# rslmtoasa/rslmtoasa

Hardware: AMD Instinct MI355X
Metric: block-recursion throughput (H|psi> + A_n + B_n recursion levels, recursion.f90 recur_b) (higher is better)
Workload: dtype f64

## Files before the change

### rslmtoasa_amd/csrc/kernels_spmm5.hpp

```cpp
#pragma once
#include <hip/hip_runtime.h>
#include <algorithm>
#include <type_traits>
#include <utility>
#include <vector>
#include "kernels_valu.hpp"
#include "kernels_mfma.hpp"
#include "kernels_spmm4.hpp"

namespace rsrec {

#ifndef RSREC_S5_KSPLIT_PROBE
#define RSREC_S5_KSPLIT_PROBE 0
#endif
#ifndef RSREC_S5_PRIO
#define RSREC_S5_PRIO 0
#endif
#ifndef RSREC_S5_GRAM_STRIP_LOADS
#define RSREC_S5_GRAM_STRIP_LOADS 0
#endif
#ifndef S5_WG_GROUPS
#define S5_WG_GROUPS 4
#endif
constexpr int S5_TRIPLE = 640;
// ... 182 lines not shown
                if ((int)E.size() > nextra) {
                    Head& H = head_main[(size_t)set * ntau + tau];
                    H.blk.assign(E[nextra].blk, E[nextra].blk + 2 * BLK); H.flip = 0; H.valid = true;
                }
                for (int sig = 0; sig < 2; ++sig)
                    emit_stream(E, sig, 0, (9 * (int)E.size() + 9) / 10, host.data() + set * per_set + ((size_t)tau * 2 + sig) * per_sig);
            }
        if (hipMemcpy(d_frag, host.data(), host.size() * sizeof(double), hipMemcpyHostToDevice) != hipSuccess) return "upload of spmm5 fragments failed";
        return nullptr;
    }
    void emit_head(int set, int tau, const double* extra, double* out) const {
        const Head& H = head_main[(size_t)set * ntau + tau];
        std::vector<Entry> E = {{extra, nslots, 0}, {extra, nslots, 1}};
        if (H.valid) E.push_back({H.blk.data(), 0, H.flip});
        for (int sig = 0; sig < 2; ++sig) emit_stream(E, sig, 0, S5_HEAD_TRIPLES, out + (size_t)sig * S5_HEAD_TRIPLES * S5_TRIPLE);
    }
    const char* build(int nslots_lat, int hstride, int ntype, int nmax, int hoh, const double* st, const double* loc, const double* eeo, const double* hallo,
                      const double* enim, const double* lsham, const int* iz0, const double* const* dev = nullptr, hipStream_t stream = nullptr) {
        const int nt = nmax + ntype, nset = hoh ? 2 : 1, nfs = nslots_lat + 1;
        const size_t B = 2 * (size_t)BLK;
        std::vector<const double*> blk((size_t)nset * nt * nfs, nullptr);
        const size_t tmp_per = dev ? 1 : (size_t)nfs;
        std::vector<double> tmp((size_t)(hoh ? nt : 0) * tmp_per * B, 0.0);
        std::vector<S5Desc> desc(dev ? (size_t)nset * nt * nfs : 0, S5Desc{nullptr, nullptr, 1.0, 0.0});
        for (int tau = 0; tau < nt; ++tau)
            for (int s = 0; s < nslots_lat; ++s) {
                const size_t off = tau < nmax ? B * (s + (size_t)hstride * tau) : B * (s + (size_t)hstride * (tau - nmax));
                const double* h0 = (tau < nmax ? loc : st) + off;
                blk[(size_t)tau * nfs + s] = h0;
                if (dev) desc[(size_t)tau * nfs + s] = S5Desc{(tau < nmax ? dev[1] : dev[0]) + off, nullptr, 1.0, 0.0};
                if (hoh) {
                    const double* ho = (tau < nmax ? hallo : eeo) + off;
                    if (dev) { blk[((size_t)nt + tau) * nfs + s] = ho; desc[((size_t)nt + tau) * nfs + s] = S5Desc{(tau < nmax ? dev[3] : dev[2]) + off, nullptr, -1.0, s == 0 ? 1.0 : 0.0}; }
                    else {
                        double* d = tmp.data() + B * ((size_t)tau * tmp_per + s);
                        for (size_t e = 0; e < B; ++e) d[e] = -ho[e];
                        if (s == 0) for (int q = 0; q < NB; ++q) d[2 * (q + NB * q)] += 1.0;
                        blk[((size_t)nt + tau) * nfs + s] = d;
                    }
                }
            }
        if (hoh)
            for (int tau = 0; tau < nt; ++tau) {
                const int ty = tau < nmax ? iz0[tau] : tau - nmax;
                double* d = tmp.data() + B * ((size_t)tau * tmp_per + (dev ? 0 : nslots_lat));
                for (size_t e = 0; e < B; ++e) d[e] = enim[B * ty + e] + lsham[B * ty + e];
                blk[((size_t)nt + tau) * nfs + nslots_lat] = d;
                if (dev) desc[((size_t)nt + tau) * nfs + nslots_lat] = S5Desc{dev[4] + B * ty, dev[5] + B * ty, 1.0, 0.0};
            }
        if (!dev) return build_custom(nslots_lat, nt, nset, blk);
        if (const char* msg = make_schedule(nslots_lat, nt, nset, kinds_of(blk), nullptr)) return msg;
        head_main.assign((size_t)nset * nt, Head());
        const size_t dneed = desc.size() * sizeof(S5Desc);
        if (dneed > desc_bytes) {
            if (d_desc) (void)hipFree(d_desc);
            d_desc = nullptr; desc_bytes = 0;
            if (hipMalloc(reinterpret_cast<void**>(&d_desc), dneed) != hipSuccess) return "hipMalloc of spmm5 block descriptors failed";
            desc_bytes = dneed;
        }
        if (hipMemcpyAsync(d_desc, desc.data(), dneed, hipMemcpyHostToDevice, stream) != hipSuccess) return "upload of spmm5 block descriptors failed";
        if (hipStreamSynchronize(stream) != hipSuccess) return "upload of spmm5 block descriptors failed";
        k_s5_emit<<<dim3(ntr, 2, nset * nt), S5_TRIPLE, 0, stream>>>(d_desc, d_meta, META, nfs, nslots_lat + 1, ntr, d_frag);
        if (hipGetLastError() != hipSuccess) return "launch of the operator-stream assembly failed";
        return nullptr;
    }
    int single_class(int set) const {
        int one = -1;
        for (int tau = 0; tau < ntau; ++tau)
            if (ksteps[(size_t)set * ntau + tau] > 0) { if (one >= 0) return -1; one = tau; }
        return one;
    }
    double required_flops(int set, int tau, int slot) const {
        const size_t q = ((size_t)set * ntau + tau) * (nslots + 1) + slot;
        if (q >= mixing.size() || mixing[q] < 0) return 0.0;
        return mixing[q] ? 46656.0 : 23328.0;
    }
    double flops_per_group(int set, int tau) const { return ksteps.empty() ? 0.0 : 2.0 * ksteps[(size_t)set * ntau + tau] * 9.0 * (2.0 * 16 * 16 * 4 + 2.0 * 4 * 4 * 4 * 4); }
    const double* frag_set(int set) const { return d_frag + (size_t)set * ntau * 2 * ntr * S5_TRIPLE; }
    const int* meta_set(int set) const { return d_meta + (size_t)set * ntau * META; }
};

typedef double s5_d2 __attribute__((ext_vector_type(2)));
struct S5Pair { s5_d2 b[9]; s5_d2 a[2]; };
struct S5Single { double b[9]; double a[2]; };
struct S5Acc { double4_t m[9]; double r[9]; };

struct S5Ent { unsigned off[GROUP]; unsigned rem; };

template <int S> struct S5St {
    static constexpr int T = S / 3, K = S % 3;
    static constexpr int W = K == 2 ? 2 : 4;
    static constexpr int o0 = 10 * T + (K == 0 ? 0 : K == 1 ? 4 : 8);
    static constexpr int eA = o0 / 9, mA0 = o0 % 9, sp = 9 - mA0;
    static constexpr bool straddle = sp < W;
    static constexpr bool opens = straddle || mA0 == 0;
    static constexpr int eOpen = mA0 == 0 ? eA : eA + 1;
};

template <int NL, int NM>
__device__ __forceinline__ void s5_interleave() {
    constexpr int PER = NM / NL;
#pragma unroll
    for (int i = 0; i < NL; ++i) {
        __builtin_amdgcn_sched_group_barrier(0x20, 1, 0);
        __builtin_amdgcn_sched_group_barrier(0x8, PER, 0);
    }
    __builtin_amdgcn_sched_group_barrier(0x8, NM - PER * NL, 0);
}

template <int NL = 11>
__device__ __forceinline__ void s5_mfma(S5Acc& acc, const S5Pair& o) {
#pragma unroll
    for (int e = 0; e < 2; ++e)
#pragma unroll
        for (int t = 0; t < 9; ++t) {
            acc.m[t] = __builtin_amdgcn_mfma_f64_16x16x4f64(o.a[0][e], o.b[t][e], acc.m[t], 0, 0, 0);
            acc.r[t] = __builtin_amdgcn_mfma_f64_4x4x4f64(o.a[1][e], o.b[t][e], acc.r[t], 0, 0, 0);
        }
    s5_interleave<NL, 36>();
}
template <int NL = 11>
__device__ __forceinline__ void s5_mfma(S5Acc& acc, const S5Single& o) {
#pragma unroll
    for (int t = 0; t < 9; ++t) {
        acc.m[t] = __builtin_amdgcn_mfma_f64_16x16x4f64(o.a[0], o.b[t], acc.m[t], 0, 0, 0);
        acc.r[t] = __builtin_amdgcn_mfma_f64_4x4x4f64(o.a[1], o.b[t], acc.r[t], 0, 0, 0);
    }
    s5_interleave<NL, 18>();
}

template <int N> using S5C = std::integral_constant<int, N>;
template <int T0, int... I, class F>
__device__ __forceinline__ void s5_each_tile(std::integer_sequence<int, I...>, F&& f) { (f(S5C<T0 + I>{}, S5C<I>{}), ...); }
template <int SRC>
__device__ __forceinline__ s5_d2 s5_row_bcast(s5_d2 v) {
    s5_d2 r;
#pragma unroll
    for (int c = 0; c < 2; ++c) {
        const int lo = __builtin_amdgcn_update_dpp(0, __double2loint(v[c]), 0x150 + SRC , 0xf, 0xf, true);
        const int hi = __builtin_amdgcn_update_dpp(0, __double2hiint(v[c]), 0x150 + SRC, 0xf, 0xf, true);
        r[c] = __hiloint2double(hi, lo);
    }
    return r;
}
#define S5_GLOBAL __attribute__((address_space(1)))
#define S5_CONST __attribute__((address_space(4)))
#define S5_LDS __attribute__((address_space(3)))
typedef const S5_GLOBAL char* s5_gp;

template <bool TWO, bool LDSA, bool OCT = false>
__device__ __forceinline__ void s5_run_stream(S5Acc& acc, const int* __restrict__ meta, const char* __restrict__ fr , const char* __restrict__ fr_head,
                                              const char* __restrict__ inb, const char* __restrict__ in2b,
                                              const int* __restrict__ nbr5 ,
                                              const int (&atom)[GROUP] , int rem_sel ,
                                              int ncol, int sig, int l4,
                                              unsigned lane_main, unsigned lane_z, unsigned lane_rem, unsigned lane_rem_z, unsigned lane16, unsigned lane8,
                                              const int (&tile_blk)[GROUP], int rem_blk , int kpart = 0) {
    int left = meta[0];
    int ebase = 0, tbase = 0;
    bool first = true;
#if RSREC_S5_KSPLIT_PROBE
    if (kpart == 0) left = min(left, 27);
    else { left -= 27; ebase = 10; tbase = 9; first = false; }
#endif
    if (left <= 0) return;
    const bool extras = TWO && meta[1] != 0;
    const S5_CONST int* codes = (const S5_CONST int*)(meta + 2);
    const S5_CONST int* nbr = (const S5_CONST int*)nbr5;
    S5Ent E0, E1;
    int raw[GROUP];
    int code_cur = codes[ebase], code_nxt = codes[ebase + 1];
    auto load_idx = [&](int col) {
#pragma unroll
        for (int t = 0; t < GROUP; ++t) raw[t] = nbr[(size_t)ncol * atom[t] + col];
    };
    load_idx(code_cur & 255);
    unsigned vlane_main = lane_main, vlane_z = lane_z, vlane16 = lane16, vlane8 = lane8;
    auto open_entry = [&](int j, S5Ent& E) {
        const unsigned so = 2592u * (unsigned)((code_cur >> 8) ? 1 - sig : sig);
#pragma unroll
        for (int t = 0; t < GROUP; ++t) E.off[t] = (unsigned)(OCT ? raw[t] + tile_blk[t] : raw[t]) * (BLD * 8u) + so;
        const int r01 = (rem_sel & 1) ? raw[1] : raw[0], r23 = (rem_sel & 1) ? raw[3] : raw[2], r45 = (rem_sel & 1) ? raw[5] : raw[4], r67 = (rem_sel & 1) ? raw[7] : raw[6];
        const int r03 = (rem_sel & 2) ? r23 : r01, r47 = (rem_sel & 2) ? r67 : r45;
        E.rem = (unsigned)(((rem_sel & 4) ? r47 : r03) + (OCT ? rem_blk : 0)) * (BLD * 8u) + so;
        code_cur = code_nxt;
        code_nxt = codes[j + 2];
        load_idx(code_cur & 255);
    };
    auto issue = [&](auto s2c, auto& o) {
        constexpr int S2 = decltype(s2c)::value, S = S2 % 27, wrap = S2 / 27;
        using I = S5St<S>;
        S5Ent& EA = (I::eA & 1) ? E1 : E0;
        S5Ent& EB = (I::eA & 1) ? E0 : E1;
        if constexpr (I::opens) open_entry(ebase + 10 * wrap + I::eOpen, (I::eOpen & 1) ? E1 : E0);
        const bool head = wrap == 0 && first && extras;
        const char* __restrict__ base = (TWO && S < 5 && head) ? in2b : inb;
        s5_gp fbg = nullptr;
        if constexpr (!LDSA) {
            const char* fb = ((TWO && I::T < S5_HEAD_TRIPLES && head && fr_head) ? fr_head + I::T * S5_TRIPLE_BYTES
                                                                                 : fr + (size_t)(tbase + 9 * wrap + I::T) * S5_TRIPLE_BYTES)
                             + (I::K == 0 ? 0 : I::K == 1 ? 2048 : 4096);
            fbg = (s5_gp)fb;
            asm("" : "+s"(fbg));
        }
        constexpr unsigned rowA = 288u * I::mA0, rowB = 0u - 288u * I::sp;
        unsigned& lm = I::K < 2 ? vlane_main : vlane_z;
        unsigned& lf = I::K < 2 ? vlane16 : vlane8;
        const unsigned lr = I::K < 2 ? lane_rem : lane_rem_z;
        asm volatile("" : "+v"(lm));
        asm volatile("" : "+v"(lf));
        using V = std::remove_reference_t<decltype(o.b[0])>;
        if constexpr (!I::straddle) {
#pragma unroll
            for (int t = 0; t < GROUP; ++t) {
                s5_gp pt = (s5_gp)base + EA.off[t];
                asm("" : "+s"(pt));
                o.b[t] = *(const S5_GLOBAL V*)(pt + lm + rowA);
            }
            o.b[8] = *(const S5_GLOBAL V*)((s5_gp)base + (EA.rem + lr) + rowA);
        } else {
            const bool inB = (I::K < 2 ? l4 : (l4 >> 1)) >= I::sp;
#pragma unroll
            for (int t = 0; t < GROUP; ++t) {
                const unsigned off = (inB ? EB.off[t] + rowB : EA.off[t] + rowA) + lm;
                o.b[t] = *(const S5_GLOBAL V*)((s5_gp)base + off);
            }
            const unsigned off = (inB ? EB.rem + rowB : EA.rem + rowA) + lr;
            o.b[8] = *(const S5_GLOBAL V*)((s5_gp)base + off);
        }
        if constexpr (LDSA) {
            const S5_LDS char* fl = (const S5_LDS char*)fr + (unsigned)(tbase + 9 * wrap + I::T) * S5_TRIPLE_BYTES + (I::K == 0 ? 0 : I::K == 1 ? 2048 : 4096);
#pragma unroll
            for (int q = 0; q < 2; ++q) o.a[q] = *(const S5_LDS V*)(fl + lf + q * (I::K < 2 ? 1024 : 512));
        } else if constexpr (I::K < 2) {
#pragma unroll
            for (int q = 0; q < 2; ++q) o.a[q] = *(const S5_GLOBAL V*)(fbg + lf + q * 1024);
        } else {
#pragma unroll
            for (int q = 0; q < 2; ++q) o.a[q] = *(const S5_GLOBAL V*)(fbg + lf + q * 512);
        }
    };
    S5Pair X, Y;
    S5Single Z;
    issue(S5C<0>{}, X);
    issue(S5C<1>{}, Y);
#define S5_STEP(S, NEXT, CUR)                 \
    if (left > (S)) {                         \
        issue(S5C<(S) + 2>{}, NEXT);          \
        s5_mfma<LDSA ? 9 : 11>(acc, CUR);     \
        __builtin_amdgcn_sched_barrier(0);    \
    }
    for (;; left -= 27) {
        S5_STEP(0, Z, X) S5_STEP(1, X, Y) S5_STEP(2, Y, Z) S5_STEP(3, Z, X) S5_STEP(4, X, Y) S5_STEP(5, Y, Z)
        S5_STEP(6, Z, X) S5_STEP(7, X, Y) S5_STEP(8, Y, Z) S5_STEP(9, Z, X) S5_STEP(10, X, Y) S5_STEP(11, Y, Z)
        S5_STEP(12, Z, X) S5_STEP(13, X, Y) S5_STEP(14, Y, Z) S5_STEP(15, Z, X) S5_STEP(16, X, Y) S5_STEP(17, Y, Z)
        S5_STEP(18, Z, X) S5_STEP(19, X, Y) S5_STEP(20, Y, Z) S5_STEP(21, Z, X) S5_STEP(22, X, Y) S5_STEP(23, Y, Z)
        S5_STEP(24, Z, X) S5_STEP(25, X, Y) S5_STEP(26, Y, Z)
        if (left <= 27) break;
        ebase += 10; tbase += 9; first = false;
    }
#undef S5_STEP
}


template <int NT> struct S5PairN { s5_d2 b[NT]; s5_d2 a[2]; };
template <int NT> struct S5SingleN { double b[NT]; double a[2]; };
template <int NT> struct S5AccN { double4_t m[NT]; double r[NT]; };

template <int NT>
__device__ __forceinline__ void s5_mfma_n(S5AccN<NT>& acc, const S5PairN<NT>& o) {
#pragma unroll
    for (int e = 0; e < 2; ++e)
#pragma unroll
        for (int t = 0; t < NT; ++t) {
            acc.m[t] = __builtin_amdgcn_mfma_f64_16x16x4f64(o.a[0][e], o.b[t][e], acc.m[t], 0, 0, 0);
            acc.r[t] = __builtin_amdgcn_mfma_f64_4x4x4f64(o.a[1][e], o.b[t][e], acc.r[t], 0, 0, 0);
        }
    s5_interleave<NT, 4 * NT>();
}
template <int NT>
__device__ __forceinline__ void s5_mfma_n(S5AccN<NT>& acc, const S5SingleN<NT>& o) {
#pragma unroll
    for (int t = 0; t < NT; ++t) {
        acc.m[t] = __builtin_amdgcn_mfma_f64_16x16x4f64(o.a[0], o.b[t], acc.m[t], 0, 0, 0);
        acc.r[t] = __builtin_amdgcn_mfma_f64_4x4x4f64(o.a[1], o.b[t], acc.r[t], 0, 0, 0);
    }
    s5_interleave<NT, 2 * NT>();
}

struct S5EntN { unsigned off[3]; unsigned rem; };

template <bool TWO, int NMAIN, bool HASREM>
__device__ __forceinline__ void s5_run_stream_n(S5AccN<NMAIN + (HASREM ? 1 : 0)>& acc, const int* __restrict__ meta, const char* __restrict__ fr ,
                                                const char* __restrict__ inb, const char* __restrict__ in2b, const int* __restrict__ nbr5,
                                                const int (&atom)[NMAIN], const int (&ratom)[GROUP], int rem_sel, int ncol, int sig, int l4,
                                                unsigned lane_main, unsigned lane_z, unsigned lane_rem, unsigned lane_rem_z, unsigned lane16, unsigned lane8) {
    constexpr int NT = NMAIN + (HASREM ? 1 : 0);
    int left = meta[0];
    int ebase = 0, tbase = 0;
    bool first = true;
    if (left <= 0) return;
    const bool extras = TWO && meta[1] != 0;
    const S5_CONST int* codes = (const S5_CONST int*)(meta + 2);
    const S5_CONST int* nbr = (const S5_CONST int*)nbr5;
    S5EntN E0, E1;
    int raw[NMAIN], rraw[GROUP];
    int code_cur = codes[ebase], code_nxt = codes[ebase + 1];
    auto load_idx = [&](int col) {
#pragma unroll
        for (int t = 0; t < NMAIN; ++t) raw[t] = nbr[(size_t)ncol * atom[t] + col];
        if constexpr (HASREM) {
#pragma unroll
            for (int t = 0; t < GROUP; ++t) rraw[t] = nbr[(size_t)ncol * ratom[t] + col];
        }
    };
    load_idx(code_cur & 255);
    unsigned vlane_main = lane_main, vlane_z = lane_z, vlane16 = lane16, vlane8 = lane8;
    auto open_entry = [&](int j, S5EntN& E) {
        const unsigned so = 2592u * (unsigned)((code_cur >> 8) ? 1 - sig : sig);
#pragma unroll
        for (int t = 0; t < NMAIN; ++t) E.off[t] = (unsigned)raw[t] * (BLD * 8u) + so;
        if constexpr (HASREM) {
            const int r01 = (rem_sel & 1) ? rraw[1] : rraw[0], r23 = (rem_sel & 1) ? rraw[3] : rraw[2], r45 = (rem_sel & 1) ? rraw[5] : rraw[4], r67 = (rem_sel & 1) ? rraw[7] : rraw[6];
            const int r03 = (rem_sel & 2) ? r23 : r01, r47 = (rem_sel & 2) ? r67 : r45;
            E.rem = (unsigned)((rem_sel & 4) ? r47 : r03) * (BLD * 8u) + so;
        }
        code_cur = code_nxt;
        code_nxt = codes[j + 2];
        load_idx(code_cur & 255);
    };
    auto issue = [&](auto s2c, auto& o) {
        constexpr int S2 = decltype(s2c)::value, S = S2 % 27, wrap = S2 / 27;
        using I = S5St<S>;
        S5EntN& EA = (I::eA & 1) ? E1 : E0;
        S5EntN& EB = (I::eA & 1) ? E0 : E1;
        if constexpr (I::opens) open_entry(ebase + 10 * wrap + I::eOpen, (I::eOpen & 1) ? E1 : E0);
        const bool head = wrap == 0 && first && extras;
        const char* __restrict__ base = (TWO && S < 5 && head) ? in2b : inb;
        constexpr unsigned rowA = 288u * I::mA0, rowB = 0u - 288u * I::sp;
        unsigned& lm = I::K < 2 ? vlane_main : vlane_z;
        unsigned& lf = I::K < 2 ? vlane16 : vlane8;
        const unsigned lr = I::K < 2 ? lane_rem : lane_rem_z;
        asm volatile("" : "+v"(lm));
        asm volatile("" : "+v"(lf));
        using V = std::remove_reference_t<decltype(o.b[0])>;
        if constexpr (!I::straddle) {
#pragma unroll
            for (int t = 0; t < NMAIN; ++t) {
                s5_gp pt = (s5_gp)base + EA.off[t];
                asm("" : "+s"(pt));
                o.b[t] = *(const S5_GLOBAL V*)(pt + lm + rowA);
            }
            if constexpr (HASREM) o.b[NMAIN] = *(const S5_GLOBAL V*)((s5_gp)base + (EA.rem + lr) + rowA);
        } else {
            const bool inB = (I::K < 2 ? l4 : (l4 >> 1)) >= I::sp;
#pragma unroll
            for (int t = 0; t < NMAIN; ++t) {
                const unsigned off = (inB ? EB.off[t] + rowB : EA.off[t] + rowA) + lm;
                o.b[t] = *(const S5_GLOBAL V*)((s5_gp)base + off);
            }
            if constexpr (HASREM) {
                const unsigned off = (inB ? EB.rem + rowB : EA.rem + rowA) + lr;
                o.b[NMAIN] = *(const S5_GLOBAL V*)((s5_gp)base + off);
            }
        }
        const S5_LDS char* fl = (const S5_LDS char*)fr + (unsigned)(tbase + 9 * wrap + I::T) * S5_TRIPLE_BYTES + (I::K == 0 ? 0 : I::K == 1 ? 2048 : 4096);
#pragma unroll
        for (int q = 0; q < 2; ++q) o.a[q] = *(const S5_LDS V*)(fl + lf + q * (I::K < 2 ? 1024 : 512));
    };
    S5PairN<NT> X0, Y0, X1, Y1;
    S5SingleN<NT> Z0, Z1;
    issue(S5C<0>{}, X0);
    issue(S5C<1>{}, Y0);
    issue(S5C<2>{}, Z0);
    issue(S5C<3>{}, X1);
    issue(S5C<4>{}, Y1);
#define S5_STEP(S, NEXT, CUR)                 \
    if (left > (S)) {                         \
        issue(S5C<(S) + 5>{}, NEXT);          \
        s5_mfma_n<NT>(acc, CUR);              \
        __builtin_amdgcn_sched_barrier(0);    \
    }
    for (;; left -= 54) {
        S5_STEP(0, Z1, X0) S5_STEP(1, X0, Y0) S5_STEP(2, Y0, Z0) S5_STEP(3, Z0, X1) S5_STEP(4, X1, Y1) S5_STEP(5, Y1, Z1)
        S5_STEP(6, Z1, X0) S5_STEP(7, X0, Y0) S5_STEP(8, Y0, Z0) S5_STEP(9, Z0, X1) S5_STEP(10, X1, Y1) S5_STEP(11, Y1, Z1)
        S5_STEP(12, Z1, X0) S5_STEP(13, X0, Y0) S5_STEP(14, Y0, Z0) S5_STEP(15, Z0, X1) S5_STEP(16, X1, Y1) S5_STEP(17, Y1, Z1)
        S5_STEP(18, Z1, X0) S5_STEP(19, X0, Y0) S5_STEP(20, Y0, Z0) S5_STEP(21, Z0, X1) S5_STEP(22, X1, Y1) S5_STEP(23, Y1, Z1)
        S5_STEP(24, Z1, X0) S5_STEP(25, X0, Y0) S5_STEP(26, Y0, Z0) S5_STEP(27, Z0, X1) S5_STEP(28, X1, Y1) S5_STEP(29, Y1, Z1)
        S5_STEP(30, Z1, X0) S5_STEP(31, X0, Y0) S5_STEP(32, Y0, Z0) S5_STEP(33, Z0, X1) S5_STEP(34, X1, Y1) S5_STEP(35, Y1, Z1)
        S5_STEP(36, Z1, X0) S5_STEP(37, X0, Y0) S5_STEP(38, Y0, Z0) S5_STEP(39, Z0, X1) S5_STEP(40, X1, Y1) S5_STEP(41, Y1, Z1)
        S5_STEP(42, Z1, X0) S5_STEP(43, X0, Y0) S5_STEP(44, Y0, Z0) S5_STEP(45, Z0, X1) S5_STEP(46, X1, Y1) S5_STEP(47, Y1, Z1)
        S5_STEP(48, Z1, X0) S5_STEP(49, X0, Y0) S5_STEP(50, Y0, Z0) S5_STEP(51, Z0, X1) S5_STEP(52, X1, Y1) S5_STEP(53, Y1, Z1)
        if (left <= 54) break;
        ebase += 20; tbase += 18; first = false;
    }
#undef S5_STEP
}

struct S5Epilogue { int kind = 0; const double* cur = nullptr; const double* old = nullptr; double a = 1.0, b = 0.0; };

struct S5Gram { double* out = nullptr; size_t cstride = 0; long min_groups = 0; };

template <bool TWO, bool LDSA, bool OCT = false, int NSP = 1, bool GRAM = false>
__global__ __launch_bounds__(NSP == 3 ? 768 : S5_WG_GROUPS * 128) void k_spmm5(SpmmDims D, const int* __restrict__ order_all, const int* __restrict__ cum,
                                               const int* __restrict__ nbr ,
                                               const int* __restrict__ izp, const double* __restrict__ frag, const int* __restrict__ meta, int ntr,
                                               const double* __restrict__ in_all, double* __restrict__ out_all,
                                               const double* __restrict__ in2_all = nullptr,
                                               const double* __restrict__ frag_head = nullptr ,
                                               int ntau = 0, int lds_tau = 0 ,
                                               int* __restrict__ queue = nullptr ,
                                               int spin_by_xcd = 1 ,
                                               S5Epilogue epi = S5Epilogue(), S5Gram gram = S5Gram()) {
    static_assert(!GRAM || (!TWO && !OCT && NSP == 1), "the Gram epilogue: one input, whole groups of atoms");
    extern __shared__ double s5_lds[];
    const int lane = threadIdx.x & 63;
    const int wave = __builtin_amdgcn_readfirstlane(threadIdx.x >> 6);
    const int sig = LDSA ? (int)((spin_by_xcd ? blockIdx.x : (blockIdx.x >> 3)) & 1) : wave / S5_WG_GROUPS, gslot = LDSA ? wave : wave % S5_WG_GROUPS;
#if RSREC_S5_PRIO
    if (wave >= (int)(blockDim.x >> 7)) __builtin_amdgcn_s_setprio(1);
#endif
    const int WGG = LDSA ? (int)(blockDim.x >> 6) : S5_WG_GROUPS;
    int bxl = blockIdx.x, gdxl = gridDim.x, run_lo = D.run_lo, run_hi = D.run_hi, qrun = 0;
    if (LDSA && D.nruns > 0) {
        const int row = spin_by_xcd ? 8 : 16, rowi = (int)blockIdx.x / row;
        int r = 0;
#pragma unroll
        for (int q = 1; q < 4; ++q) if (q < D.nruns && rowi >= D.run_row0[q]) r = q;
        lds_tau = D.run_tau[r]; run_lo = D.run_glo[r]; run_hi = D.run_ghi[r];
        bxl = (int)blockIdx.x - row * D.run_row0[r];
        gdxl = row * (D.run_row0[r + 1] - D.run_row0[r]);
        qrun = r;
    }
    if constexpr (LDSA) {
        const s5_d2* __restrict__ src = reinterpret_cast<const s5_d2*>(frag + ((size_t)lds_tau * 2 + sig) * ntr * S5_TRIPLE);
        s5_d2* dst = reinterpret_cast<s5_d2*>(s5_lds);
        const int n = ntr * (S5_TRIPLE / 2);
        constexpr int PER = (int)(160 * 1024 / 16 / (NSP == 3 ? 512 : S5_WG_GROUPS * 64));
        const int nthr = (int)blockDim.x;
        s5_d2 v[PER];
#pragma unroll
        for (int i = 0; i < PER; ++i) { const int e = threadIdx.x + i * nthr; if (e < n) v[i] = src[e]; }
#pragma unroll
        for (int i = 0; i < PER; ++i) { const int e = threadIdx.x + i * nthr; if (e < n) dst[e] = v[i]; }
        __syncthreads();
    }
    const int l15 = lane & 15, l4 = lane >> 4;
    const unsigned lane_main = 8u * (36 * l4 + 2 * l15), lane_z = 8u * (36 * (l4 >> 1) + 2 * l15 + (l4 & 1));
    const unsigned lane_rem = 8u * (36 * l4 + 32 + 2 * (l15 & 1)), lane_rem_z = 8u * (36 * (l4 >> 1) + 32 + 2 * (l15 & 1) + (l4 & 1));
    const unsigned lane16 = 16u * lane, lane8 = 8u * lane;
    const int ncol = D.nslots + 2;
#pragma unroll 1
    for (int chain = OCT ? GROUP * (int)blockIdx.y : (int)blockIdx.y; chain < D.nchains; chain += OCT ? GROUP * (int)gridDim.y : (int)gridDim.y) {
    const int count = cum[(chain / D.cpo) * D.nlev + D.level];
    int ngroups = count / GROUP;
    const bool fold = GRAM && gram.out != nullptr && epi.kind == 0 && s5_gram_folds(ngroups, gram.min_groups);
    const int ob = D.obase[(chain / D.cpo) * D.nlev + D.level];
    const int* __restrict__ order = order_all + (size_t)(chain / D.cpo) * D.ostride + ob;
    const bool on_full_list = D.sat_base > 0 && ob == D.sat_base;
    if constexpr (OCT) ngroups = D.nmax;
    else if (run_hi > 0) {
        if (!on_full_list) continue;
        order += (size_t)run_lo * GROUP;
        ngroups = run_hi - run_lo;
    }
    const bool skipping = D.nskip > 0 && on_full_list;
    const size_t vo = (size_t)chain * D.vstride;
    const char* __restrict__ inb = reinterpret_cast<const char*>(in_all + vo);
    const char* __restrict__ in2b = TWO ? reinterpret_cast<const char*>(in2_all + vo) : nullptr;
    double* __restrict__ out = out_all + vo;
    const int zero_block = D.kk;

    int g, gend, gstep, glo = 0;
    bool dynamic = false;
    {
        const int bx = bxl;
        const int need = (ngroups + WGG - 1) / WGG;
        if constexpr (!LDSA) {
            const int nbx = max(1, min((int)gridDim.x, need));
            if (bx >= nbx) continue;
            if (nbx < 8) { g = bx * WGG + gslot; gend = ngroups; gstep = nbx * WGG; }
            else {
                const int xcd = bx & 7, j = bx >> 3;
                const int per_xcd = (nbx >> 3) + ((xcd < (nbx & 7)) ? 1 : 0);
                const int chunk = (ngroups + 7) >> 3;
                const int lo = xcd * chunk;
                gend = min(ngroups, lo + chunk);
                g = lo + j * WGG + gslot;
                gstep = per_xcd * WGG;
            }
        } else {
            const int row = spin_by_xcd ? 8 : 16;
            const int nbx = max(row, min(gdxl / row * row, (2 * need + row - 1) / row * row));
            if (bx >= nbx) continue;
            const int xcd = bx & 7, j = bx >> 3;
            if (2 * need <= row) {
                const int per_spin = row / 2, idx = spin_by_xcd ? (xcd >> 1) : xcd;
                if (j >= row / 8) continue;
                g = idx * WGG + gslot; gend = ngroups; gstep = per_spin * WGG;
            } else {
                const int rows = nbx / row;
                const int nchunk = spin_by_xcd ? 4 : 8, ichunk = spin_by_xcd ? (xcd >> 1) : xcd;
                const int chunk = (ngroups + nchunk - 1) / nchunk;
                const int lo = ichunk * chunk;
                gend = min(ngroups, lo + chunk);
                g = lo + (spin_by_xcd ? j : (j >> 1)) * WGG + gslot;
                gstep = rows * WGG;
                glo = lo;
                dynamic = queue != nullptr;
            }
        }
    }
    int* __restrict__ ctr = dynamic ? queue + ((size_t)qrun * D.nchains + chain) * 16 + 2 * (blockIdx.x & 7) + (spin_by_xcd ? 0 : sig) : nullptr;
    int part = 0;
    auto next_task = [&]() {
        if (NSP == 3 && !dynamic && part < 2) { ++part; return; }
        part = 0; g += gstep;
    };
    for (;; next_task()) {
        int kpart = 0;
        if (dynamic) {
            int gi = 0;
            if (lane == 0) gi = atomicAdd(ctr, 1);
            gi = __builtin_amdgcn_readfirstlane(gi);
#if RSREC_S5_KSPLIT_PROBE
            kpart = gi & 1; gi >>= 1;
#endif
            if constexpr (NSP == 3) { const unsigned gu = (unsigned)gi, gq = gu / 3u; part = (int)(gu - 3u * gq); gi = (int)gq; }
            g = glo + gi;
        }
        if (g >= gend) break;
        if (skipping) {
            bool skip = false;
#pragma unroll
            for (int r = 0; r < 4; ++r) skip |= r < D.nskip && g >= D.skip_lo[r] && g < D.skip_hi[r];
            if (skip) continue;
        }
        const int* __restrict__ grp = order + (size_t)g * GROUP;
        if constexpr (NSP == 3) {
            static_assert(NSP != 3 || (LDSA && !OCT), "split tasks: LDS / persistent form only");
            const int g0 = grp[0];
            const int first3 = g0 >= 0 ? g0 : zero_block;
            if (D.skip_pa && first3 < D.nmax) continue;
            const int tau3 = first3 < D.nmax ? first3 : D.nmax + izp[first3];
            const int* __restrict__ M3 = meta + (size_t)tau3 * Spmm5Operator::META;
            const char* __restrict__ fr3 = reinterpret_cast<const char*>(s5_lds);
            S5AccN<3> acc3;
#pragma unroll
            for (int t = 0; t < 3; ++t) { acc3.m[t] = (double4_t){0, 0, 0, 0}; acc3.r[t] = 0.0; }
            auto finish3 = [&](auto remc, const int (&av)[3]) {
                constexpr bool REM = decltype(remc)::value;
                size_t eo[3];
#pragma unroll
                for (int i = 0; i < 3; ++i) eo[i] = (size_t)BLD * av[i] + 324 * sig + ((REM && i == 2) ? 32 + 2 * (l15 & 1) : 2 * l15);
                s5_d2 ec[3][2], ez[3][2];
                double ecr[3], ezr[3];
                if (epi.kind) {
                    const double* cb = epi.cur + vo;
#pragma unroll
                    for (int i = 0; i < 3; ++i) {
#pragma unroll
                        for (int p = 0; p < 2; ++p) ec[i][p] = *reinterpret_cast<const s5_d2*>(cb + eo[i] + 36 * (4 * p + l4));
                        ecr[i] = cb[eo[i] + 288 + (l4 & 1)];
                    }
                    if (epi.kind == 2) {
                        const double* zb = epi.old + vo;
#pragma unroll
                        for (int i = 0; i < 3; ++i) {
#pragma unroll
                            for (int p = 0; p < 2; ++p) ez[i][p] = *reinterpret_cast<const s5_d2*>(zb + eo[i] + 36 * (4 * p + l4));
                            ezr[i] = zb[eo[i] + 288 + (l4 & 1)];
                        }
                    }
                }
#pragma unroll
                for (int i = 0; i < 3; ++i) {
                    const int a = av[i];
                    double* ob = out + eo[i];
#pragma unroll
                    for (int p = 0; p < 2; ++p) {
                        s5_d2 v; v[0] = acc3.m[i][2 * p]; v[1] = acc3.m[i][2 * p + 1];
                        if (epi.kind) {
                            v[0] = (v[0] - epi.b * ec[i][p][0]) / epi.a; v[1] = (v[1] - epi.b * ec[i][p][1]) / epi.a;
                            if (epi.kind == 2) { v[0] = v[0] * 2.0 - ez[i][p][0]; v[1] = v[1] * 2.0 - ez[i][p][1]; }
                        }
                        if (a != zero_block) *reinterpret_cast<s5_d2*>(ob + 36 * (4 * p + l4)) = v;
                    }
                    double r = acc3.r[i];
                    if (epi.kind) {
                        r = (r - epi.b * ecr[i]) / epi.a;
                        if (epi.kind == 2) r = r * 2.0 - ezr[i];
                    }
                    if (a != zero_block && l4 < 2) ob[288 + l4] = r;
                }
            };
            int ratom[GROUP];
            if (part < 2) {
                int a3[3];
#pragma unroll
                for (int j = 0; j < 3; ++j) { const int a = grp[3 * part + j]; a3[j] = a >= 0 ? a : zero_block; }
#pragma unroll
                for (int t = 0; t < GROUP; ++t) ratom[t] = zero_block;
                s5_run_stream_n<TWO, 3, false>(acc3, M3, fr3, inb, in2b, nbr, a3, ratom, 0, ncol, sig, l4, lane_main, lane_z, lane_rem, lane_rem_z, lane16, lane8);
                finish3(std::false_type{}, a3);
            } else {
#pragma unroll
                for (int t = 0; t < GROUP; ++t) { const int a = grp[t]; ratom[t] = a >= 0 ? a : zero_block; }
                const int a2[2] = {ratom[6], ratom[7]};
                int mra = grp[l15 >> 1];
                mra = mra >= 0 ? mra : zero_block;
                s5_run_stream_n<TWO, 2, true>(acc3, M3, fr3, inb, in2b, nbr, a2, ratom, l15 >> 1, ncol, sig, l4, lane_main, lane_z, lane_rem, lane_rem_z, lane16, lane8);
                const int av[3] = {a2[0], a2[1], mra};
                finish3(std::true_type{}, av);
            }
            continue;
        }
        int atom[GROUP];
        int vatom[GROUP], tile_blk[GROUP];
        int my_rem_atom, rem_blk = 0;
        if constexpr (OCT) {
            const int a0 = g;
#pragma unroll
            for (int t = 0; t < GROUP; ++t) {
                const bool ok = a0 >= 0 && chain + t < D.nchains;
                atom[t] = ok ? a0 : zero_block;
                tile_blk[t] = ok ? t * (D.kk + 1) : 0;
                vatom[t] = ok ? a0 + t * (D.kk + 1) : zero_block;
            }
            const int tr = l15 >> 1;
            const bool okr = a0 >= 0 && chain + tr < D.nchains;
            rem_blk = okr ? tr * (D.kk + 1) : 0;
            my_rem_atom = okr ? a0 + tr * (D.kk + 1) : zero_block;
        } else {
#pragma unroll
            for (int t = 0; t < GROUP; ++t) { const int a = grp[t]; atom[t] = a >= 0 ? a : zero_block; vatom[t] = atom[t]; tile_blk[t] = 0; }
            my_rem_atom = grp[l15 >> 1];
            my_rem_atom = my_rem_atom >= 0 ? my_rem_atom : zero_block;
        }
        const int first = atom[0];
        if (!OCT && D.skip_pa && first < D.nmax) continue;
        const int tau = first < D.nmax ? first : D.nmax + izp[first];
        const int* __restrict__ M = meta + (size_t)tau * Spmm5Operator::META;
        const char* __restrict__ fr = LDSA ? reinterpret_cast<const char*>(s5_lds) : reinterpret_cast<const char*>(frag + ((size_t)tau * 2 + sig) * ntr * S5_TRIPLE);
        const char* __restrict__ fh = (TWO && frag_head) ? reinterpret_cast<const char*>(frag_head + ((size_t)chain * ntau + tau) * S5_HEAD_DOUBLES + (size_t)sig * S5_HEAD_TRIPLES * S5_TRIPLE) : nullptr;

        S5Acc acc;
#pragma unroll
        for (int t = 0; t < 9; ++t) { acc.m[t] = (double4_t){0, 0, 0, 0}; acc.r[t] = 0.0; }

        if constexpr (OCT) s5_run_stream<TWO, LDSA, true>(acc, M, fr, fh, inb, in2b, nbr, atom, l15 >> 1, ncol, sig, l4, lane_main, lane_z, lane_rem, lane_rem_z, lane16, lane8, tile_blk, rem_blk);
        else s5_run_stream<TWO, LDSA>(acc, M, fr, fh, inb, in2b, nbr, atom, l15 >> 1, ncol, sig, l4, lane_main, lane_z, lane_rem, lane_rem_z, lane16, lane8, tile_blk, rem_blk, kpart);
#if RSREC_S5_KSPLIT_PROBE
        if (kpart) continue;
#endif

        int fl15 = l15, fl4 = l4;
        if constexpr (GRAM) {
            unsigned fl;
            asm volatile("v_mbcnt_lo_u32_b32 %0, -1, 0\n\tv_mbcnt_hi_u32_b32 %0, -1, %0" : "=v"(fl));
            fl15 = (int)fl & 15; fl4 = (int)fl >> 4;
        }
        const int ekind = GRAM ? 0 : epi.kind;
        auto finish = [&](auto t0c, auto t1c) {
            constexpr int T0 = decltype(t0c)::value, T1 = decltype(t1c)::value, NT = T1 - T0;
            size_t eo[NT];
#pragma unroll
            for (int i = 0; i < NT; ++i) { const int t = T0 + i; eo[i] = (size_t)BLD * ((t < 8) ? vatom[t] : my_rem_atom) + 324 * sig + ((t < 8) ? 2 * fl15 : 32 + 2 * (fl15 & 1)); }
            s5_d2 ec[NT][2], ez[NT][2];
            double ecr[NT], ezr[NT];
            if (ekind) {
                const double* cb = epi.cur + vo;
#pragma unroll
                for (int i = 0; i < NT; ++i) {
#pragma unroll
                    for (int p = 0; p < 2; ++p) ec[i][p] = *reinterpret_cast<const s5_d2*>(cb + eo[i] + 36 * (4 * p + fl4));
                    ecr[i] = cb[eo[i] + 288 + (fl4 & 1)];
                }
                if (ekind == 2) {
                    const double* zb = epi.old + vo;
#pragma unroll
                    for (int i = 0; i < NT; ++i) {
#pragma unroll
                        for (int p = 0; p < 2; ++p) ez[i][p] = *reinterpret_cast<const s5_d2*>(zb + eo[i] + 36 * (4 * p + fl4));
                        ezr[i] = zb[eo[i] + 288 + (fl4 & 1)];
                    }
                }
            }
#pragma unroll
            for (int i = 0; i < NT; ++i) {
                const int t = T0 + i;
                const int a = (t < 8) ? vatom[t] : my_rem_atom;
                double* ob = out + eo[i];
#pragma unroll
                for (int p = 0; p < 2; ++p) {
                    s5_d2 v; v[0] = acc.m[t][2 * p]; v[1] = acc.m[t][2 * p + 1];
                    if (ekind) {
                        v[0] = (v[0] - epi.b * ec[i][p][0]) / epi.a; v[1] = (v[1] - epi.b * ec[i][p][1]) / epi.a;
                        if (ekind == 2) { v[0] = v[0] * 2.0 - ez[i][p][0]; v[1] = v[1] * 2.0 - ez[i][p][1]; }
                    }
                    if (a != zero_block) *reinterpret_cast<s5_d2*>(ob + 36 * (4 * p + fl4)) = v;
                }
                double r = acc.r[t];
                if (ekind) {
                    r = (r - epi.b * ecr[i]) / epi.a;
                    if (ekind == 2) r = r * 2.0 - ezr[i];
                }
                if (a != zero_block && fl4 < 2) ob[288 + fl4] = r;
            }
        };
        bool stored = false;
        if constexpr (GRAM) if (fold) {
            unsigned gl;
            asm volatile("v_mbcnt_lo_u32_b32 %0, -1, 0\n\tv_mbcnt_hi_u32_b32 %0, -1, %0" : "=v"(gl));
            const int lane = (int)gl, l15 = lane & 15, l4 = lane >> 4;
            const double* __restrict__ ub = in_all + vo;
            double4_t gre = {0, 0, 0, 0}, gim = {0, 0, 0, 0};
            double sre[2] = {0.0, 0.0}, sim[2] = {0.0, 0.0}, kre[2] = {0.0, 0.0}, kim[2] = {0.0, 0.0};
            auto rem_coef = [&](s5_d2 u, double& cr, double& ci) {
                cr = l4 == 0 ? u[0] : (l4 == 1 ? u[1] : 0.0);
                ci = l4 == 0 ? -u[1] : (l4 == 1 ? u[0] : 0.0);
            };
            constexpr bool STRIP_LOADS = RSREC_S5_GRAM_STRIP_LOADS != 0;
            auto strip_loads = [&](s5_d2 (&gs)[3][2], const double* ab) {
#pragma unroll
                for (int p = 0; p < 3; ++p)
#pragma unroll
                    for (int e = 0; e < 2; ++e) gs[p][e] = *reinterpret_cast<const s5_d2*>(ab + 36 * (p < 2 ? 4 * p + l4 : 8) + 32 + 2 * e);
            };
            s5_d2 gs8[3][2];
            if constexpr (!STRIP_LOADS) strip_loads(gs8, ub + (size_t)BLD * my_rem_atom + 324 * sig);
            auto gram_tiles = [&](auto t0c, auto t1c) {
                constexpr int T0 = decltype(t0c)::value, T1 = decltype(t1c)::value, NT = T1 - T0;
                s5_d2 gu[NT][3], gs[STRIP_LOADS ? NT : 1][3][2];
#pragma unroll
                for (int i = 0; i < NT; ++i) {
                    const int t = T0 + i;
                    const double* ab = ub + (size_t)BLD * ((t < 8) ? vatom[t] : my_rem_atom) + 324 * sig;
#pragma unroll
                    for (int p = 0; p < 3; ++p)
                        if (t < 8) gu[i][p] = *reinterpret_cast<const s5_d2*>(ab + 36 * (p < 2 ? 4 * p + l4 : 8) + 2 * l15);
                    if constexpr (STRIP_LOADS) strip_loads(gs[i], ab);
                }
                if constexpr (!STRIP_LOADS && T0 == 0) {
                    __builtin_amdgcn_sched_barrier(0);
                    finish(S5C<0>{}, S5C<5>{});
                    finish(S5C<5>{}, S5C<9>{});
                    stored = true;
                    __builtin_amdgcn_sched_barrier(0);
                }
                s5_each_tile<T0>(std::make_integer_sequence<int, NT>{}, [&](auto tc, auto ic) {
                    constexpr int t = decltype(tc)::value, i = decltype(ic)::value;
                    const double x8 = acc.r[t];
                    if constexpr (t < 8) {
#pragma unroll
                        for (int p = 0; p < 2; ++p) {
                            gre = __builtin_amdgcn_mfma_f64_16x16x4f64(gu[i][p][0], acc.m[t][2 * p], gre, 0, 0, 0);
                            gre = __builtin_amdgcn_mfma_f64_16x16x4f64(gu[i][p][1], acc.m[t][2 * p + 1], gre, 0, 0, 0);
                            gim = __builtin_amdgcn_mfma_f64_16x16x4f64(-gu[i][p][1], acc.m[t][2 * p], gim, 0, 0, 0);
                            gim = __builtin_amdgcn_mfma_f64_16x16x4f64(gu[i][p][0], acc.m[t][2 * p + 1], gim, 0, 0, 0);
                        }
                        double cr, ci;
                        rem_coef(gu[i][2], cr, ci);
                        gre = __builtin_amdgcn_mfma_f64_16x16x4f64(cr, x8, gre, 0, 0, 0);
                        gim = __builtin_amdgcn_mfma_f64_16x16x4f64(ci, x8, gim, 0, 0, 0);
                    }
                    auto strip = [&](int p, int e) -> s5_d2 {
                        if constexpr (STRIP_LOADS) return gs[i][p][e];
                        else if constexpr (t < 8) return s5_row_bcast<2 * t>(gs8[p][e]);
                        else return gs8[p][e];
                    };
                    double (&are)[2] = (t < 8) ? sre : kre;
                    double (&aim)[2] = (t < 8) ? sim : kim;
#pragma unroll
                    for (int e = 0; e < 2; ++e) {
#pragma unroll
                        for (int p = 0; p < 2; ++p) {
                            const s5_d2 u = strip(p, e);
                            const double ur = u[0], ui = u[1], tr = acc.m[t][2 * p], ti = acc.m[t][2 * p + 1];
                            are[e] = fma(ur, tr, are[e]); are[e] = fma(ui, ti, are[e]);
                            aim[e] = fma(ur, ti, aim[e]); aim[e] = fma(-ui, tr, aim[e]);
                        }
                        double cr, ci;
                        rem_coef(strip(2, e), cr, ci);
                        are[e] = fma(cr, x8, are[e]);
                        aim[e] = fma(ci, x8, aim[e]);
                    }
                });
                if constexpr (!STRIP_LOADS) {
                    if constexpr (T0 < 8) asm volatile("" : "+v"(sre[0]), "+v"(sre[1]), "+v"(sim[0]), "+v"(sim[1]));
                    if constexpr (T1 == 9) asm volatile("" : "+v"(kre[0]), "+v"(kre[1]), "+v"(kim[0]), "+v"(kim[1]));
                }
            };
            if constexpr (STRIP_LOADS) {
                gram_tiles(S5C<0>{}, S5C<2>{});
                __builtin_amdgcn_sched_barrier(0);
                gram_tiles(S5C<2>{}, S5C<4>{});
                __builtin_amdgcn_sched_barrier(0);
                gram_tiles(S5C<4>{}, S5C<6>{});
                __builtin_amdgcn_sched_barrier(0);
                gram_tiles(S5C<6>{}, S5C<8>{});
                __builtin_amdgcn_sched_barrier(0);
                gram_tiles(S5C<8>{}, S5C<9>{});
            } else {
                gram_tiles(S5C<0>{}, S5C<4>{});
// ... 42 lines not shown
```

### rslmtoasa_amd/csrc/kernels_uscheme.hpp

```cpp
#pragma once
#include "kernels_mfma.hpp"
#include "kernels_spmm5.hpp"

namespace rsrec {

__host__ __device__ constexpr int pk_col(int q, int l4) { return q < 8 ? 8 * (q >> 1) + 2 * l4 + (q & 1) : 32 + l4; }

__device__ __forceinline__ void emit_rhs_frags_pk(const double2* M, double sign, double* out, int ci_layout) {
    for (int e = threadIdx.x; e < 27 * 64; e += blockDim.x) {
        const int l = e & 63, qf = e >> 6, q = qf / 3, f = qf % 3;
        const int ki = pk_col(q, l >> 4);
        const int ko = (f < 2) ? 16 * f + (l & 15) : 32 + (l & 3);
        const int pi = ci_layout ? (ki & 1) : ki / 18, ci = ci_layout ? (ki >> 1) : ki % 18;
        const int po = ci_layout ? (ko & 1) : ko / 18, co = ci_layout ? (ko >> 1) : ko % 18;
        const double2 g = M[ci + 18 * co];
        const double v = (pi == po) ? g.x : (pi == 0 ? g.y : -g.y);
        out[e] = sign * v;
    }
}

__device__ __forceinline__ void matmul18(const double2* A, const double2* B, double2* C) {
    for (int e = threadIdx.x; e < BLK; e += blockDim.x) {
        const int i = e % NB, j = e / NB;
        double2 acc = make_double2(0.0, 0.0);
        for (int k = 0; k < NB; ++k) {
            const double2 a = A[i + NB * k], b = B[k + NB * j];
            acc.x += a.x * b.x - a.y * b.y;
            acc.y += a.x * b.y + a.y * b.x;
        }
        C[e] = acc;
    }
}

struct U3Operands { double2 x[4]; double2 y; };

__device__ __forceinline__ void u3_load(U3Operands& o, const double* __restrict__ base, unsigned off, int l4) {
    const double2* p = reinterpret_cast<const double2*>(base + off + 2 * l4);
#pragma unroll
    for (int qq = 0; qq < 4; ++qq) o.x[qq] = ld_stream(p + 4 * qq);
    o.y = ld_stream(reinterpret_cast<const double2*>(base + off + 32 + 2 * (l4 >> 1)));
}

template <int Q>
__device__ __forceinline__ double u3_k(const U3Operands& o, bool odd) { return Q < 8 ? ((Q & 1) ? o.x[Q >> 1].y : o.x[Q >> 1].x) : (odd ? o.y.y : o.y.x); }

__device__ __forceinline__ void u3_mac(double4_t& ca, double4_t& cb, double& cr, const U3Operands& o, const double (&T)[27], bool odd) {
#define U3_STEP(Q)                                                                              \
    {                                                                                           \
        const double a = u3_k<Q>(o, odd);                                                          \
        ca = __builtin_amdgcn_mfma_f64_16x16x4f64(a, T[3 * (Q) + 0], ca, 0, 0, 0);              \
        cb = __builtin_amdgcn_mfma_f64_16x16x4f64(a, T[3 * (Q) + 1], cb, 0, 0, 0);              \
        cr = __builtin_amdgcn_mfma_f64_4x4x4f64(a, T[3 * (Q) + 2], cr, 0, 0, 0);                \
    }
    U3_STEP(0) U3_STEP(1) U3_STEP(2) U3_STEP(3) U3_STEP(4) U3_STEP(5) U3_STEP(6) U3_STEP(7) U3_STEP(8)
#undef U3_STEP
}

__global__ __launch_bounds__(MF_WAVES * 64, 1) void k_mfma_orth3(ChainView CV, int level, int zero_block, const double* __restrict__ tvec,
                                                                const double* __restrict__ ucur, double* uprev,
                                                                const double* __restrict__ tabs, double* partial ,
                                                                double* unext = nullptr ) {
    __shared__ double lds[MF_WAVES * 1296];
    const int chain = blockIdx.y;
    const int lane = threadIdx.x & 63;
    const int wave = __builtin_amdgcn_readfirstlane(threadIdx.x >> 6);
    const int ngroups = CV.count_of(chain, level) / GROUP;
    const int* order = CV.order_of(chain, level);
    const size_t vo = (size_t)chain * CV.vstride;
    const double* tv = tvec + vo;
    const double* uc = ucur + vo;
    double* up = uprev + vo;
    double* uo = (unext ? unext : uprev) + vo;
    const int l15 = lane & 15, l4 = lane >> 4, l3 = lane & 3, lg = (lane >> 2) & 3;
    double T1[27], T2[27], T3[27];
    {
        const double* f = tabs + (size_t)chain * 3 * 27 * 64 + lane;
#pragma unroll
        for (int e = 0; e < 27; ++e) { T1[e] = f[e * 64]; T2[e] = f[(27 + e) * 64]; T3[e] = f[(54 + e) * 64]; }
    }
    GramAcc Gm;
    Gm.zero();
    const int nbx = active_workgroups(ngroups);
    GroupWalk w((int)blockIdx.x < nbx ? ngroups : 0, wave, nbx);
    const int ntile = (w.g < w.end) ? ((w.end - w.g + w.step - 1) / w.step) * 9 : 0;
    struct TileAtoms { int s0, a_lo, a_hi; };
    auto tile_atoms = [&](int it) {
        it = min(it, ntile - 1);
        const int* __restrict__ grp = order + (size_t)(w.g + (it / 9) * w.step) * GROUP;
        TileAtoms t;
        t.s0 = (16 * (it % 9)) / 18;
        t.a_lo = grp[t.s0];
        t.a_hi = grp[min(t.s0 + 1, GROUP - 1)];
        return t;
    };
    auto tile_row = [&](const TileAtoms& t, int rho) {
        const bool hi = rho >= 18 * (t.s0 + 1);
        const int a = hi ? t.a_hi : t.a_lo;
        RowRef R;
        R.valid = a >= 0;
        R.off = (unsigned)BLD * (unsigned)(R.valid ? a : zero_block) + 36u * (unsigned)(rho - 18 * (t.s0 + (hi ? 1 : 0)));
        return R;
    };
    auto load_tile = [&](int it, U3Operands& a, U3Operands& c, U3Operands& p) {
        const TileAtoms t = tile_atoms(it);
        const RowRef ra = tile_row(t, 16 * (min(it, ntile - 1) % 9) + l15);
        u3_load(a, tv, ra.off, l4);
        u3_load(c, uc, ra.off, l4);
        u3_load(p, up, ra.off, l4);
    };
    struct Pending { double4_t ca, cb; double cr; TileAtoms ta; int mt; };
    Pending P;
    bool pending = false;
    auto retire = [&](const double (&fr)[4]) {
#pragma unroll
        for (int j = 0; j < 4; ++j) {
            const RowRef rs = tile_row(P.ta, 16 * P.mt + l4 + 4 * j);
            if (rs.valid) { st_stream(uo + rs.off + l15, (double)P.ca[j]); st_stream(uo + rs.off + 16 + l15, (double)P.cb[j]); }
        }
        const RowRef rr = tile_row(P.ta, 16 * P.mt + 4 * lg + l4);
        if (rr.valid) st_stream(uo + rr.off + 32 + l3, P.cr);
#pragma unroll
        for (int j = 0; j < 4; ++j) {
            const double f0 = P.ca[j], f1 = P.cb[j];
            Gm.t00 = __builtin_amdgcn_mfma_f64_16x16x4f64(f0, f0, Gm.t00, 0, 0, 0);
            Gm.t01 = __builtin_amdgcn_mfma_f64_16x16x4f64(f0, f1, Gm.t01, 0, 0, 0);
            Gm.t11 = __builtin_amdgcn_mfma_f64_16x16x4f64(f1, f1, Gm.t11, 0, 0, 0);
            Gm.tr0 = __builtin_amdgcn_mfma_f64_4x4x4f64(fr[j], f0, Gm.tr0, 0, 0, 0);
            Gm.tr1 = __builtin_amdgcn_mfma_f64_4x4x4f64(fr[j], f1, Gm.tr1, 0, 0, 0);
            Gm.trr = __builtin_amdgcn_mfma_f64_4x4x4f64(fr[j], fr[j], Gm.trr, 0, 0, 0);
        }
    };
    auto compute_tile = [&](int it, const U3Operands& ot, const U3Operands& oc, const U3Operands& op) {
        double fr[4] = {0.0, 0.0, 0.0, 0.0};
        if (pending) {
#pragma unroll
            for (int j = 0; j < 4; ++j) fr[j] = __shfl(P.cr, l3 + 4 * j + 16 * l4, 64);
        }
        Pending N;
        N.ta = tile_atoms(it);
        N.mt = it % 9;
        N.ca = (double4_t){0, 0, 0, 0}; N.cb = (double4_t){0, 0, 0, 0}; N.cr = 0.0;
        u3_mac(N.ca, N.cb, N.cr, ot, T1, l4 & 1);
        if (pending) retire(fr);
        u3_mac(N.ca, N.cb, N.cr, op, T2, l4 & 1);
        u3_mac(N.ca, N.cb, N.cr, oc, T3, l4 & 1);
        P = N;
        pending = true;
    };
    U3Operands at, ac, ap, bt, bc, bp, ct, cc, cp;
    if (ntile > 0) { load_tile(0, at, ac, ap); load_tile(1, bt, bc, bp); }
#pragma unroll 1
    for (int it = 0; it < ntile; it += 3) {
        load_tile(it + 2, ct, cc, cp);
        __builtin_amdgcn_sched_barrier(0);
        compute_tile(it, at, ac, ap);
        __builtin_amdgcn_sched_barrier(0);
        if (it + 1 < ntile) {
            load_tile(it + 3, at, ac, ap);
            __builtin_amdgcn_sched_barrier(0);
            compute_tile(it + 1, bt, bc, bp);
            __builtin_amdgcn_sched_barrier(0);
        }
        if (it + 2 < ntile) {
            load_tile(it + 4, bt, bc, bp);
            __builtin_amdgcn_sched_barrier(0);
            compute_tile(it + 2, ct, cc, cp);
            __builtin_amdgcn_sched_barrier(0);
        }
    }
    if (pending) {
        double fr[4];
#pragma unroll
        for (int j = 0; j < 4; ++j) fr[j] = __shfl(P.cr, l3 + 4 * j + 16 * l4, 64);
        retire(fr);
    }
    gram_block_out(Gm, lds, partial + ((size_t)chain * gridDim.x + blockIdx.x) * 1296, true);
}

template <int F>
__device__ __forceinline__ void u3_mac_lds(double4_t& ca, double4_t& cb, double& cr, const U3Operands& o, const double* __restrict__ T , bool odd) {
#define U3L_STEP(Q)                                                                             \
    {                                                                                           \
        const double a = u3_k<Q>(o, odd);                                                          \
        ca = __builtin_amdgcn_mfma_f64_16x16x4f64(a, T[(3 * (Q) + 0) * 64], ca, 0, 0, 0);       \
        cb = __builtin_amdgcn_mfma_f64_16x16x4f64(a, T[(3 * (Q) + 1) * 64], cb, 0, 0, 0);       \
        cr = __builtin_amdgcn_mfma_f64_4x4x4f64(a, T[(3 * (Q) + 2) * 64], cr, 0, 0, 0);         \
    }
    U3L_STEP(0) U3L_STEP(1) U3L_STEP(2) U3L_STEP(3) U3L_STEP(4) U3L_STEP(5) U3L_STEP(6) U3L_STEP(7) U3L_STEP(8)
#undef U3L_STEP
}

__global__ __launch_bounds__(MF_WAVES * 64, 2) void k_mfma_orth3w(ChainView CV, int level, int zero_block, const double* __restrict__ tvec,
                                                                 const double* __restrict__ ucur, double* uprev,
                                                                 const double* __restrict__ tabs, double* partial ) {
    __shared__ double lds[MF_WAVES * 1296];
    const int chain = blockIdx.y;
    const int lane = threadIdx.x & 63;
    const int wave = __builtin_amdgcn_readfirstlane(threadIdx.x >> 6);
    const int ngroups = CV.count_of(chain, level) / GROUP;
    const int* order = CV.order_of(chain, level);
    const size_t vo = (size_t)chain * CV.vstride;
    const double* tv = tvec + vo;
    const double* uc = ucur + vo;
    double* up = uprev + vo;
    const int l15 = lane & 15, l4 = lane >> 4, l3 = lane & 3, lg = (lane >> 2) & 3;
    {
        const double* f = tabs + (size_t)chain * 3 * 27 * 64;
        for (int e = threadIdx.x; e < 3 * 27 * 64; e += MF_WAVES * 64) lds[e] = f[e];
        __syncthreads();
    }
    const double* T1 = lds + lane;
    const double* T2 = lds + 27 * 64 + lane;
    const double* T3 = lds + 54 * 64 + lane;
    GramAcc Gm;
    Gm.zero();
    const int nbx = active_workgroups(ngroups);
    GroupWalk w((int)blockIdx.x < nbx ? ngroups : 0, wave, nbx);
    const int ntile = (w.g < w.end) ? ((w.end - w.g + w.step - 1) / w.step) * 9 : 0;
    struct TileAtoms { int s0, a_lo, a_hi; };
    auto tile_atoms = [&](int it) {
        it = min(it, ntile - 1);
        const int* __restrict__ grp = order + (size_t)(w.g + (it / 9) * w.step) * GROUP;
        TileAtoms t;
        t.s0 = (16 * (it % 9)) / 18;
        t.a_lo = grp[t.s0];
        t.a_hi = grp[min(t.s0 + 1, GROUP - 1)];
        return t;
    };
    auto tile_row = [&](const TileAtoms& t, int rho) {
        const bool hi = rho >= 18 * (t.s0 + 1);
        const int a = hi ? t.a_hi : t.a_lo;
        RowRef R;
        R.valid = a >= 0;
        R.off = (unsigned)BLD * (unsigned)(R.valid ? a : zero_block) + 36u * (unsigned)(rho - 18 * (t.s0 + (hi ? 1 : 0)));
        return R;
    };
    auto load_tile = [&](int it, U3Operands& a, U3Operands& c, U3Operands& p) {
        const TileAtoms t = tile_atoms(it);
        const RowRef ra = tile_row(t, 16 * (min(it, ntile - 1) % 9) + l15);
        u3_load(a, tv, ra.off, l4);
        u3_load(c, uc, ra.off, l4);
        u3_load(p, up, ra.off, l4);
    };
    auto compute_tile = [&](int it, const U3Operands& ot, const U3Operands& oc, const U3Operands& op) {
        const TileAtoms ta = tile_atoms(it);
        const int mt = it % 9;
        double4_t ca = (double4_t){0, 0, 0, 0}, cb = (double4_t){0, 0, 0, 0};
        double cr = 0.0;
        u3_mac_lds<0>(ca, cb, cr, ot, T1, l4 & 1);
        u3_mac_lds<1>(ca, cb, cr, op, T2, l4 & 1);
        u3_mac_lds<2>(ca, cb, cr, oc, T3, l4 & 1);
#pragma unroll
        for (int j = 0; j < 4; ++j) {
            const RowRef rs = tile_row(ta, 16 * mt + l4 + 4 * j);
            if (rs.valid) { up[rs.off + l15] = ca[j]; up[rs.off + 16 + l15] = cb[j]; }
        }
        const RowRef rr = tile_row(ta, 16 * mt + 4 * lg + l4);
        if (rr.valid) up[rr.off + 32 + l3] = cr;
#pragma unroll
        for (int j = 0; j < 4; ++j) {
            const double fr = __shfl(cr, l3 + 4 * j + 16 * l4, 64);
            const double f0 = ca[j], f1 = cb[j];
            Gm.t00 = __builtin_amdgcn_mfma_f64_16x16x4f64(f0, f0, Gm.t00, 0, 0, 0);
            Gm.t01 = __builtin_amdgcn_mfma_f64_16x16x4f64(f0, f1, Gm.t01, 0, 0, 0);
            Gm.t11 = __builtin_amdgcn_mfma_f64_16x16x4f64(f1, f1, Gm.t11, 0, 0, 0);
            Gm.tr0 = __builtin_amdgcn_mfma_f64_4x4x4f64(fr, f0, Gm.tr0, 0, 0, 0);
            Gm.tr1 = __builtin_amdgcn_mfma_f64_4x4x4f64(fr, f1, Gm.tr1, 0, 0, 0);
            Gm.trr = __builtin_amdgcn_mfma_f64_4x4x4f64(fr, fr, Gm.trr, 0, 0, 0);
        }
    };
    U3Operands at, ac, ap, bt, bc, bp;
    if (ntile > 0) load_tile(0, at, ac, ap);
#pragma unroll 1
    for (int it = 0; it < ntile; it += 2) {
        load_tile(it + 1, bt, bc, bp);
        __builtin_amdgcn_sched_barrier(0);
        compute_tile(it, at, ac, ap);
        __builtin_amdgcn_sched_barrier(0);
        if (it + 1 < ntile) {
            load_tile(it + 2, at, ac, ap);
            __builtin_amdgcn_sched_barrier(0);
            compute_tile(it + 1, bt, bc, bp);
            __builtin_amdgcn_sched_barrier(0);
        }
    }
    __syncthreads();
    gram_block_out(Gm, lds, partial + ((size_t)chain * gridDim.x + blockIdx.x) * 1296, true);
}

__global__ __launch_bounds__(1024) void k_reduce_a_u(const double* __restrict__ partial, int nblk, double2* a_out, size_t astride,
                                                    const double2* __restrict__ Bmats , double* tabs, int ci) {
    __shared__ double lds[1296];
    __shared__ double2 Gm[BLK], Bi[BLK], M1[BLK], M2[BLK];
    const int chain = blockIdx.x;
    const double2 c = reduce_gram(partial + (size_t)chain * nblk * 1296, nblk, lds, ci);
    if (threadIdx.x < BLK) { Gm[threadIdx.x] = c; Bi[threadIdx.x] = Bmats[(size_t)chain * 2 * BLK + BLK + threadIdx.x]; }
    __syncthreads();
    matmul18(Gm, Bi, M1);
    __syncthreads();
    matmul18(Bi, M1, M2);
    __syncthreads();
    if (threadIdx.x < BLK) a_out[chain * astride + threadIdx.x] = M2[threadIdx.x];
    matmul18(Bi, M2, M1);
    __syncthreads();
    emit_rhs_frags_pk(M1, -1.0, tabs + ((size_t)chain * 3 + 2) * 27 * 64, ci);
}

__global__ __launch_bounds__(1024) void k_reduce_b_u(const double* __restrict__ partial, int nblk, double2* b2_out, size_t bstride, double2* Bmats,
                                                    double* tabs, int* status, int ci) {
    __shared__ double lds[1296];
    __shared__ Eig18Shared sh;
    __shared__ double2 Bn[BLK], Bin[BLK], Bold[BLK], M1[BLK];
    const int chain = blockIdx.x;
    const double2 c = reduce_gram(partial + (size_t)chain * nblk * 1296, nblk, lds, ci);
    double2* Bout = Bmats + (size_t)chain * 2 * BLK;
    if (threadIdx.x < BLK) { b2_out[chain * bstride + threadIdx.x] = c; sh.A[threadIdx.x] = c; Bold[threadIdx.x] = Bout[BLK + threadIdx.x]; }
    __syncthreads();
    const int sw = jacobi18(sh);
    if (sw < 0 && threadIdx.x == 0) atomicOr(status, 1);
    if (threadIdx.x < NB) { const double l = sqrt(sh.ev[threadIdx.x]); sh.f1[threadIdx.x] = l; sh.f2[threadIdx.x] = 1.0 / l; }
    __syncthreads();
    matfun18(sh, sh.f1, Bn);
    matfun18(sh, sh.f2, Bin);
    __syncthreads();
    matmul18(Bold, Bn, M1);
    for (int e = threadIdx.x; e < BLK; e += blockDim.x) { Bout[e] = Bn[e]; Bout[BLK + e] = Bin[e]; }
    __syncthreads();
    emit_rhs_frags_pk(Bin, 1.0, tabs + ((size_t)chain * 3 + 0) * 27 * 64, ci);
    emit_rhs_frags_pk(M1, -1.0, tabs + ((size_t)chain * 3 + 1) * 27 * 64, ci);
}

__global__ void k_uscheme_init(double2* Bmats, double* tabs, int ci) {
    __shared__ double2 I[BLK];
    const int chain = blockIdx.x;
    for (int e = threadIdx.x; e < BLK; e += blockDim.x) I[e] = make_double2((e % NB) == (e / NB) ? 1.0 : 0.0, 0.0);
    __syncthreads();
    for (int e = threadIdx.x; e < 2 * BLK; e += blockDim.x) Bmats[(size_t)chain * 2 * BLK + e] = I[e % BLK];
    emit_rhs_frags_pk(I, 1.0, tabs + ((size_t)chain * 3 + 0) * 27 * 64, ci);
    for (int e = threadIdx.x; e < 2 * 27 * 64; e += blockDim.x) tabs[((size_t)chain * 3 + 1) * 27 * 64 + e] = 0.0;
}


#ifndef CHEB_UNROLL
#define CHEB_UNROLL 4
#endif
template <bool FIRST, bool FUSED = false>
__global__ __launch_bounds__(MF_WAVES * 64, 2) void k_mfma_cheb(ChainView CV, int level, int zero_block, const double* __restrict__ tvec,
                                                               const double* __restrict__ cur_all, const double* __restrict__ old_all,
                                                               double* __restrict__ out_all, double a, double b, double* partial) {
    __shared__ double lds[MF_WAVES * 1296];
    const int chain = blockIdx.y;
    const int lane = threadIdx.x & 63;
    const int wave = __builtin_amdgcn_readfirstlane(threadIdx.x >> 6);
    const int ngroups = CV.count_of(chain, level) / GROUP;
    const int* order = CV.order_of(chain, level);
    const size_t vo = (size_t)chain * CV.vstride;
    const double* tv = FUSED ? nullptr : tvec + vo;
    const double* cu = cur_all + vo;
    const double* ol = (FIRST || FUSED) ? nullptr : old_all + vo;
    double* out = out_all + vo;
    const int l15 = lane & 15, l4 = lane >> 4, l3 = lane & 3, lg = (lane >> 2) & 3;
    GramAcc G1, G2;
    G1.zero(); G2.zero();
    const int nbx = active_workgroups(ngroups);
    for (GroupWalk w((int)blockIdx.x < nbx ? ngroups : 0, wave, nbx); w.g < w.end; w.g += w.step) {
        const int* grp = order + (size_t)w.g * GROUP;
#pragma unroll CHEB_UNROLL
        for (int kq = 0; kq < 36; ++kq) {
            const RowRef rk = group_row(grp, 4 * kq + l4, zero_block);
            const double c0 = cu[rk.off + l15], c1 = cu[rk.off + 16 + l15], cr = cu[rk.off + 32 + l3];
            double n0, n1, nr;
            if (FUSED) {
                n0 = out[rk.off + l15]; n1 = out[rk.off + 16 + l15]; nr = out[rk.off + 32 + l3];
            } else {
                const double t0 = tv[rk.off + l15], t1 = tv[rk.off + 16 + l15], tr = tv[rk.off + 32 + l3];
                n0 = (t0 - b * c0) / a; n1 = (t1 - b * c1) / a; nr = (tr - b * cr) / a;
                if (!FIRST) {
                    const double z0 = ol[rk.off + l15], z1 = ol[rk.off + 16 + l15], zr = ol[rk.off + 32 + l3];
                    n0 = n0 * 2.0 - z0; n1 = n1 * 2.0 - z1; nr = nr * 2.0 - zr;
                }
                if (rk.valid) {
                    out[rk.off + l15] = n0; out[rk.off + 16 + l15] = n1;
                    if (lg == 0) out[rk.off + 32 + l3] = nr;
                }
            }
            if (FIRST) {
                G2.t00 = __builtin_amdgcn_mfma_f64_16x16x4f64(c0, n0, G2.t00, 0, 0, 0);
                G2.t01 = __builtin_amdgcn_mfma_f64_16x16x4f64(c0, n1, G2.t01, 0, 0, 0);
                G2.t10 = __builtin_amdgcn_mfma_f64_16x16x4f64(c1, n0, G2.t10, 0, 0, 0);
                G2.t11 = __builtin_amdgcn_mfma_f64_16x16x4f64(c1, n1, G2.t11, 0, 0, 0);
                G2.tr0 = __builtin_amdgcn_mfma_f64_4x4x4f64(cr, n0, G2.tr0, 0, 0, 0);
                G2.tr1 = __builtin_amdgcn_mfma_f64_4x4x4f64(cr, n1, G2.tr1, 0, 0, 0);
                G2.t0r = __builtin_amdgcn_mfma_f64_4x4x4f64(c0, nr, G2.t0r, 0, 0, 0);
                G2.t1r = __builtin_amdgcn_mfma_f64_4x4x4f64(c1, nr, G2.t1r, 0, 0, 0);
                G2.trr = __builtin_amdgcn_mfma_f64_4x4x4f64(cr, nr, G2.trr, 0, 0, 0);
            } else {
                G1.t00 = __builtin_amdgcn_mfma_f64_16x16x4f64(c0, c0, G1.t00, 0, 0, 0);
                G1.t01 = __builtin_amdgcn_mfma_f64_16x16x4f64(c0, c1, G1.t01, 0, 0, 0);
                G1.t11 = __builtin_amdgcn_mfma_f64_16x16x4f64(c1, c1, G1.t11, 0, 0, 0);
                G1.tr0 = __builtin_amdgcn_mfma_f64_4x4x4f64(cr, c0, G1.tr0, 0, 0, 0);
                G1.tr1 = __builtin_amdgcn_mfma_f64_4x4x4f64(cr, c1, G1.tr1, 0, 0, 0);
                G1.trr = __builtin_amdgcn_mfma_f64_4x4x4f64(cr, cr, G1.trr, 0, 0, 0);
                G2.t00 = __builtin_amdgcn_mfma_f64_16x16x4f64(n0, c0, G2.t00, 0, 0, 0);
                G2.t01 = __builtin_amdgcn_mfma_f64_16x16x4f64(n0, c1, G2.t01, 0, 0, 0);
                G2.t10 = __builtin_amdgcn_mfma_f64_16x16x4f64(n1, c0, G2.t10, 0, 0, 0);
                G2.t11 = __builtin_amdgcn_mfma_f64_16x16x4f64(n1, c1, G2.t11, 0, 0, 0);
                G2.tr0 = __builtin_amdgcn_mfma_f64_4x4x4f64(nr, c0, G2.tr0, 0, 0, 0);
                G2.tr1 = __builtin_amdgcn_mfma_f64_4x4x4f64(nr, c1, G2.tr1, 0, 0, 0);
                G2.t0r = __builtin_amdgcn_mfma_f64_4x4x4f64(n0, cr, G2.t0r, 0, 0, 0);
                G2.t1r = __builtin_amdgcn_mfma_f64_4x4x4f64(n1, cr, G2.t1r, 0, 0, 0);
                G2.trr = __builtin_amdgcn_mfma_f64_4x4x4f64(nr, cr, G2.trr, 0, 0, 0);
// ... 65 lines not shown
```

### rslmtoasa_amd/csrc/rsrec.hip

```cpp
#include <hip/hip_runtime.h>
#include <hsa/hsa.h>
#include <hsa/hsa_ext_amd.h>
#include <dlfcn.h>
#include <algorithm>
#include <array>
#include <atomic>
#include <chrono>
#include <cmath>
#include <cstdarg>
#include <cstdio>
#include <cstdlib>
#include <cstring>
#include <memory>
#include <string>
#include <thread>
#include <tuple>
#include <vector>

#include "../../include/rsrec.h"
#include "kernels_valu.hpp"
#include "kernels_mfma.hpp"
#include "kernels_spmm4.hpp"
#include "kernels_spmm5.hpp"
#include "kernels_uscheme.hpp"
#include "kernels_green.hpp"
#include "kernels_ldos.hpp"
#include "kernels_spectra.hpp"
#include "kernels_moments.hpp"
#include "kernels_kubo.hpp"
#include "kernels_cond.hpp"
#include "kernels_optical.hpp"
#include "kernels_exchange.hpp"
#include "kernels_auxgreen.hpp"
#include "kernels_contour.hpp"
#include "kernels_assemble.hpp"
#include "kernels_fan.hpp"
#include "kernels_bloch.hpp"

using namespace rsrec;

namespace {

struct DevBuf {
    void* p = nullptr;
    size_t bytes = 0;
    DevBuf() = default;
    DevBuf(DevBuf&& o) noexcept : p(o.p), bytes(o.bytes) { o.p = nullptr; o.bytes = 0; }
    DevBuf& operator=(DevBuf&& o) noexcept { std::swap(p, o.p); std::swap(bytes, o.bytes); return *this; }
    ~DevBuf() { release(); }
    hipError_t reserve(size_t n) {
        if (n <= bytes) return hipSuccess;
        release();
        hipError_t e = hipMalloc(&p, n);
        if (e == hipSuccess) bytes = n;
        return e;
    }
    void release() { if (p) (void)hipFree(p); p = nullptr; bytes = 0; }
    template <class T> T* as() const { return reinterpret_cast<T*>(p); }
};

}

struct rsrec_handle {
    int device = 0;
    hipStream_t stream = nullptr;
    hipStream_t copy_stream = nullptr;
    hipEvent_t ev_green[2] = {nullptr, nullptr};
    hipStream_t side_stream = nullptr;
    hipEvent_t ev_orth = nullptr, ev_bred = nullptr;
    hipStream_t oct_stream = nullptr;
    hipEvent_t ev_oct_in = nullptr, ev_oct_out = nullptr;
    size_t p2_slot = 0;
    std::string err;
    bool have_lattice = false, have_ham = false;
    std::vector<int32_t> lat_nn, lat_iz;
    int lat_nncols = 0;
    std::vector<double> lat_cr;
    int kk = 0, nslots = 0, nmax = 0, ntype = 0;
    std::vector<int> nbr;
    std::vector<int> iz0;
    std::vector<int> radj_ptr, radj;
    DevBuf d_nbr, d_iz, d_nbr5;
    int hslots = 0, hoh = 0, nsp = 2;
    DevBuf d_hst, d_hloc, d_host, d_holoc, d_enim, d_lsham;
    Spmm4Operator s4_op;
    int s4_built_split = 0;
    Spmm5Operator s5_op;
    DevBuf d_s5queue;
    int s5_built = 0;
    size_t s5_lds_limit = (size_t)-1;
    int n_cu = 0;
    bool s4_attr = false;
    size_t term_lds = 0, cheb_ldos_lds = (size_t)64 * 1024, cheb_spec_lds = (size_t)64 * 1024;
    std::vector<double> host_ee, host_lsham, host_eeo, host_enim, host_hall, host_hallo;
    std::vector<double> host_st, host_loc;
    DevBuf d_asm[2][2], d_asm_in;
    std::vector<double> asm_host[2][2];
    int asm_nslots[2] = {0, 0}, asm_ncls[2] = {0, 0}, asm_hoh[2] = {0, 0};
    int n_octet_launch = 0;
    int n_asm_reused = 0;
    long n_asm_calls = 0, n_ldos_calls = 0, n_recursion_calls = 0;
    Spmm5Operator s5_la; int s5_la_ok = 0;
    DevBuf d_la_extra, d_rot;
    Spmm5Operator kubo_op[RSREC_KUBO_NOUT_MAX], kubo_op_b[RSREC_KUBO_NIN_MAX], kubo_hbulk;
    Spmm5Operator orb_plain;
    DevBuf d_green_in, d_green_out;
    DevBuf d_kubo[5];
    DevBuf d_cond[4];
    DevBuf d_ctens[2];
    DevBuf d_opt[5];
    DevBuf d_bsqrt, d_term, d_gim, d_ldos;
    DevBuf d_ops, d_spec;
    struct SpecImage { int nop = 0, nen = 0, n = 0, site_offset = 0, nsites_total = 0; } spec_res;
    DevBuf d_mint;
    void* pin = nullptr;
    size_t pin_bytes = 0;
    DevBuf d_frags, d_vec[6], d_partial, d_partial2, d_coefA, d_coefB, d_bmats, d_status, d_seed, d_seedcoef, d_mu, d_scal, d_zsqr;
    DevBuf d_fan, d_fan_tab, d_mpair;
    DevBuf d_bloch_geo, d_bloch_tab;
    long opt_batch = 0, opt_kernels = 0, opt_nblk = 0, opt_spmm5 = 2, opt_chain_fold = 1, opt_s5_cap = 0, opt_side = 1, opt_s5_lds = 1, opt_s5_queue = 1, opt_cheb_fused = 1;
    long opt_s5_waves = 8;
    long opt_sat_pct = 100;
    long opt_orth_oop = 1;
    long opt_s5_split = 0;
    long opt_s5_run_min = 0;
    long opt_s5_spin_xcd = 0;
    long opt_s5_octet = 8;
    long opt_s5_host_emit = 0;
    long opt_kubo_lchunk = 0;
    long opt_kubo_vbatch = 0;
    long opt_kubo_setgroup = 0;
    int n_kubo_left_chunks = 0;
    int kubo_diag_nvec = 0, kubo_diag_ll = 0;
    long opt_orth3 = 1;
    long opt_graph = 1;
    long opt_s5_gram_min = 256;
    int ham_hermitian = 0;
    std::vector<int> opp_slot;
    int opp_epoch = -1;
    DevBuf d_gram;
    double n_gram_folded = 0, n_gram_all = 0, n_gram_levels = 0;
    hipGraphExec_t graph_exec = nullptr;
    std::vector<uintptr_t> graph_key;
    bool capturing = false;
    double t_total_ms = 0, t_hop_ms = 0, t_rest_ms = 0, t_host_ms = 0;
    double t_rot_ms = 0;
    double n_hop_launch = 0, n_atom_steps = 0, n_block_mult = 0, n_hop_mfma_flop = 0;
    double n_req_flop = 0;
    int hop_fuses_a = 1;
    std::vector<hipEvent_t> ev_pool;
    size_t ev_used = 0;
    struct RegionEntry {
        std::vector<int> seeds;
        int nlev, napply, flags, epoch, ostride;
        double atom_steps, block_mults;
        DevBuf order, cum;
        std::vector<int> level_max;
        std::vector<int> hop_min, hop_max;
        std::vector<double> level_groups;
        std::vector<double> mult_hist;
        struct ClassRun { int tau, lo, hi; };
        std::vector<ClassRun> sat_runs;
        std::vector<int> level_sat;
        int sat_base = 0;
    };
    std::vector<std::unique_ptr<RegionEntry>> region_cache;
    int lattice_epoch = 0;
    const int* cur_order = nullptr;
    const int* cur_cum = nullptr;
    const std::vector<int>* cur_level_max = nullptr;
    const std::vector<double>* cur_level_groups = nullptr;
    const std::vector<double>* cur_mult_hist = nullptr;
    const RegionEntry* cur_entry = nullptr;
    int cur_nrows = 0;
    std::vector<unsigned> spatial_key;
    int res_kind = 0, res_n = 0, res_lld = 0;
    bool res_seeded = false;
    void* comm = nullptr;
    int comm_rank = 0, comm_nranks = 1;
    DevBuf d_comm;
    ~rsrec_handle();
};

namespace {

struct OptionEntry { const char* name; long rsrec_handle::*member; };
const OptionEntry OPTIONS[] = {
    {"batch", &rsrec_handle::opt_batch},
    {"kernels", &rsrec_handle::opt_kernels},
    {"nblk", &rsrec_handle::opt_nblk},
    {"spmm5", &rsrec_handle::opt_spmm5},
    {"chain_fold", &rsrec_handle::opt_chain_fold},
    {"s5_cap", &rsrec_handle::opt_s5_cap},
    {"s5_lds", &rsrec_handle::opt_s5_lds},
    {"s5_queue", &rsrec_handle::opt_s5_queue},
    {"cheb_fused", &rsrec_handle::opt_cheb_fused},
    {"side_stream", &rsrec_handle::opt_side},
    {"graph", &rsrec_handle::opt_graph},
    {"orth3", &rsrec_handle::opt_orth3},
    {"s5_waves", &rsrec_handle::opt_s5_waves},
    {"s5_split", &rsrec_handle::opt_s5_split},
    {"orth_oop", &rsrec_handle::opt_orth_oop},
    {"sat_pct", &rsrec_handle::opt_sat_pct},
    {"kubo_lchunk", &rsrec_handle::opt_kubo_lchunk},
    {"kubo_vbatch", &rsrec_handle::opt_kubo_vbatch},
    {"kubo_setgroup", &rsrec_handle::opt_kubo_setgroup},
    {"s5_host_emit", &rsrec_handle::opt_s5_host_emit},
    {"s5_octet", &rsrec_handle::opt_s5_octet},
    {"s5_spin_xcd", &rsrec_handle::opt_s5_spin_xcd},
    {"s5_run_min", &rsrec_handle::opt_s5_run_min},
    {"s5_gram_min", &rsrec_handle::opt_s5_gram_min},
};

int fail(rsrec_t* h, int code, const char* fmt, ...) {
    char buf[512];
    va_list ap;
    va_start(ap, fmt);
    vsnprintf(buf, sizeof buf, fmt, ap);
    va_end(ap);
    if (h) h->err = buf;
    return code;
}

#define HIPCK(h, call)                                                                                         \
    do {                                                                                                       \
        hipError_t e_ = (call);                                                                                \
        if (e_ != hipSuccess) return fail(h, RSREC_ERR_DEVICE, "%s failed: %s (%s:%d)", #call, hipGetErrorString(e_), __FILE__, __LINE__); \
    } while (0)

hipEvent_t next_event(rsrec_t* h) {
    static const bool off = getenv("RSREC_NO_EVENTS") != nullptr;
    if (off || h->capturing) return nullptr;
    if (h->ev_used == h->ev_pool.size()) {
        hipEvent_t e;
        if (hipEventCreate(&e) != hipSuccess) return nullptr;
        h->ev_pool.push_back(e);
    }
    hipEvent_t e = h->ev_pool[h->ev_used++];
    (void)hipEventRecord(e, h->stream);
    return e;
}

constexpr size_t PIN_BYTES = (size_t)8 << 20;
int pin_ready(rsrec_t* h) {
    if (h->pin) return RSREC_OK;
    if (hipHostMalloc(&h->pin, PIN_BYTES, hipHostMallocDefault) != hipSuccess) { h->pin = nullptr; return fail(h, RSREC_ERR_DEVICE, "hipHostMalloc of the staging buffer failed"); }
    h->pin_bytes = PIN_BYTES;
    return RSREC_OK;
}
constexpr size_t PIN_MAX_XFER = (size_t)8 << 20;
int xfer_d2h(rsrec_t* h, void* dst, const void* src_dev, size_t bytes) {
    if (bytes > PIN_MAX_XFER) {
        HIPCK(h, hipMemcpyAsync(dst, src_dev, bytes, hipMemcpyDeviceToHost, h->stream));
        HIPCK(h, hipStreamSynchronize(h->stream));
        return RSREC_OK;
    }
    int rc = pin_ready(h);
    if (rc) return rc;
    for (size_t off = 0; off < bytes; off += h->pin_bytes) {
        const size_t n = std::min(h->pin_bytes, bytes - off);
        HIPCK(h, hipMemcpyAsync(h->pin, static_cast<const char*>(src_dev) + off, n, hipMemcpyDeviceToHost, h->stream));
        HIPCK(h, hipStreamSynchronize(h->stream));
        memcpy(static_cast<char*>(dst) + off, h->pin, n);
    }
    return RSREC_OK;
}
int xfer_h2d(rsrec_t* h, void* dst_dev, const void* src, size_t bytes) {
    if (bytes > PIN_MAX_XFER) {
        HIPCK(h, hipMemcpyAsync(dst_dev, src, bytes, hipMemcpyHostToDevice, h->stream));
        HIPCK(h, hipStreamSynchronize(h->stream));
        return RSREC_OK;
    }
    int rc = pin_ready(h);
    if (rc) return rc;
    for (size_t off = 0; off < bytes; off += h->pin_bytes) {
        const size_t n = std::min(h->pin_bytes, bytes - off);
        memcpy(h->pin, static_cast<const char*>(src) + off, n);
        HIPCK(h, hipMemcpyAsync(static_cast<char*>(dst_dev) + off, h->pin, n, hipMemcpyHostToDevice, h->stream));
        HIPCK(h, hipStreamSynchronize(h->stream));
    }
    return RSREC_OK;
}
#define XFER(call) do { int rc__ = (call); if (rc__) return rc__; } while (0)

struct Region {
    std::vector<int> order;
    std::vector<int> cum;
};

void grow_region(const rsrec_t* h, const int* seeds, int nseed, int nlev, Region& R) {
    const int kk = h->kk;
    std::vector<int> dist(kk, -1);
    R.order.clear();
    R.order.reserve(kk);
    R.cum.assign(nlev, 0);
    std::vector<int> frontier, next;
    for (int s = 0; s < nseed; ++s)
        if (dist[seeds[s]] < 0) { dist[seeds[s]] = 0; frontier.push_back(seeds[s]); }
    std::sort(frontier.begin(), frontier.end());
    int level = 0;
    while (!frontier.empty() && level < nlev) {
        R.order.insert(R.order.end(), frontier.begin(), frontier.end());
        R.cum[level] = (int)R.order.size();
        next.clear();
        for (int n : frontier)
            for (int q = h->radj_ptr[n]; q < h->radj_ptr[n + 1]; ++q) {
                const int i = h->radj[q];
                if (dist[i] < 0) { dist[i] = level + 1; next.push_back(i); }
            }
        std::sort(next.begin(), next.end());
        frontier.swap(next);
        ++level;
    }
    for (int L = std::max(level, 1); L < nlev; ++L) R.cum[L] = R.cum[L - 1];
    R.order.resize(kk, 0);
}

inline unsigned spread3(unsigned v) {
    v &= 1023u;
    v = (v | (v << 16)) & 0x030000FFu;
    v = (v | (v << 8)) & 0x0300F00Fu;
    v = (v | (v << 4)) & 0x030C30C3u;
    v = (v | (v << 2)) & 0x09249249u;
    return v;
}
inline unsigned morton3(unsigned x, unsigned y, unsigned z) { return spread3(x) | (spread3(y) << 1) | (spread3(z) << 2); }

void bfs_dist(const rsrec_t* h, int start, std::vector<int>& dist) {
    const int kk = h->kk, ns = h->nslots;
    dist.assign(kk, -1);
    std::vector<int> cur{start}, nxt;
    dist[start] = 0;
    int d = 0;
    while (!cur.empty()) {
        nxt.clear();
        for (int n : cur) {
            for (int j = 1; j < ns; ++j) { const int i = h->nbr[(size_t)n * ns + j]; if (i >= 0 && dist[i] < 0) { dist[i] = d + 1; nxt.push_back(i); } }
            for (int q = h->radj_ptr[n]; q < h->radj_ptr[n + 1]; ++q) { const int i = h->radj[q]; if (dist[i] < 0) { dist[i] = d + 1; nxt.push_back(i); } }
        }
        cur.swap(nxt);
        ++d;
    }
}

void spatial_key_from_graph(rsrec_t* h) {
    const int kk = h->kk;
    std::vector<int> d0, d1, d2;
    bfs_dist(h, 0, d0);
    int l1 = 0;
    for (int i = 0; i < kk; ++i) if (d0[i] >= d0[l1]) l1 = i;
    bfs_dist(h, l1, d1);
    int l2 = 0, best = -1;
    for (int i = 0; i < kk; ++i) { const int m = std::min(d0[i], d1[i]); if (m >= best) { best = m; l2 = i; } }
    bfs_dist(h, l2, d2);
    h->spatial_key.resize(kk);
    for (int i = 0; i < kk; ++i) h->spatial_key[i] = morton3((unsigned)std::max(d0[i], 0), (unsigned)std::max(d1[i], 0), (unsigned)std::max(d2[i], 0));
}

}

extern "C" int rsrec_version(void) { return 101; }

extern "C" int rsrec_device_count(void) {
    int n = 0;
// ... 381 lines not shown
    for (const auto& e : h->region_cache)
        if (e->epoch == h->lattice_epoch && e->nlev == nlev && e->napply == napply && e->flags == flags && (int)e->seeds.size() == nb * nseed &&
            std::equal(e->seeds.begin(), e->seeds.end(), seeds0)) {
            h->cur_order = e->order.as<int>(); h->cur_cum = e->cum.as<int>(); h->cur_nrows = nb; h->cur_level_max = &e->level_max; h->cur_level_groups = &e->level_groups;
            h->cur_mult_hist = &e->mult_hist;
            h->cur_entry = e.get();
            ostride = e->ostride;
            atom_steps += e->atom_steps; block_mults += e->block_mults;
            return RSREC_OK;
        }
    const int ntau_h = h->nmax + h->ntype, nfs_h = h->nslots + 1;
    const int sat_pct = (int)std::min<long>(100, std::max<long>(1, h->opt_sat_pct));
    const int sat_from = (int)(((long)sat_pct * kk + 99) / 100);
    std::vector<Region> regs(nb);
    auto run_threads = [&](auto&& fn) {
        const int nthr = std::max(1, std::min({nb, 8, (int)std::thread::hardware_concurrency()}));
        if (nthr == 1) { for (int c = 0; c < nb; ++c) fn(c); return; }
        std::atomic<int> next_chain{0};
        std::vector<std::thread> pool;
        for (int t = 0; t < nthr; ++t)
            pool.emplace_back([&]() { for (int c = next_chain++; c < nb; c = next_chain++) fn(c); });
        for (auto& th : pool) th.join();
    };
    run_threads([&](int c) { grow_region(h, seeds0 + (size_t)c * nseed, nseed, nlev, regs[c]); });
    size_t lvneed = 8;
    for (int c = 0; c < nb; ++c) {
        size_t need = 0;
        for (int L = 0; L < nlev; ++L) {
            const int n = regs[c].cum[L];
            if (n >= sat_from || (L > 0 && n == regs[c].cum[L - 1])) continue;
            need += (size_t)n + (grouped ? (size_t)7 * std::min(ntau_h, n) + 8 : 0);
        }
        lvneed = std::max(lvneed, need);
    }
    lvneed = (lvneed + 7) / 8 * 8;
    if (lvneed + (size_t)cap > (size_t)INT32_MAX) return fail(h, RSREC_ERR_ARG, "region lists of %zu entries per chain exceed the index range", lvneed + (size_t)cap);
    if ((size_t)cap_pre + lvneed + (size_t)cap > (size_t)INT32_MAX) return fail(h, RSREC_ERR_ARG, "region lists of %zu entries per chain exceed the index range", (size_t)cap_pre + lvneed + (size_t)cap);
    const int sat_off = cap_pre + (int)lvneed;
    ostride = sat_off + cap;
    std::vector<int> order((size_t)nb * ostride, -1), cum((size_t)4 * nb * nlev, 0);
    std::vector<double> as(nb, 0.0), bm(nb, 0.0);
    const size_t hist_n = (size_t)2 * ntau_h * nfs_h;
    std::vector<double> hist((size_t)nb * hist_n, 0.0);
    auto tau = [&](int i) { return i < h->nmax ? i : h->nmax + h->iz0[i]; };
    const std::vector<unsigned>& key = h->spatial_key;
    auto before = [&](int x, int y) {
        const int tx = grouped ? tau(x) : 0, ty = grouped ? tau(y) : 0;
        if (tx != ty) return tx < ty;
        if (key[x] != key[y]) return key[x] < key[y];
        return x < y;
    };
    std::vector<int> all(kk), sat_list;
    for (int i = 0; i < kk; ++i) all[i] = i;
    std::sort(all.begin(), all.end(), before);
    sat_list.reserve(cap);
    for (int q = 0; q < kk; ++q) {
        if (grouped && q > 0 && tau(all[q]) != tau(all[q - 1])) while (sat_list.size() % GROUP) sat_list.push_back(-1);
        sat_list.push_back(all[q]);
    }
    if (grouped) while (sat_list.size() % GROUP) sat_list.push_back(-1);
    const int sat_count = (int)sat_list.size();
    std::vector<double> lgroups((size_t)nb * nlev * ntau_h, 0.0);
    auto build_chain = [&](int c) {
        const Region& R = regs[c];
        int* orow = order.data() + (size_t)c * ostride;
        int* crow = cum.data() + (size_t)c * nlev;
        int* brow = cum.data() + (size_t)(nb + c) * nlev;
        int* crow2 = cum.data() + (size_t)(2 * nb + c) * nlev;
        int* brow2 = cum.data() + (size_t)(3 * nb + c) * nlev;
        std::copy(sat_list.begin(), sat_list.end(), orow + sat_off);
        int w = cap_pre, wp = 0;
        std::vector<int> lev, region, merged;
        for (int L = 0; L < nlev; ++L) {
            const int lo = L ? R.cum[L - 1] : 0, hi = R.cum[L];
            if (hi >= sat_from) { crow[L] = crow2[L] = sat_count; brow[L] = brow2[L] = sat_off; continue; }
            lev.assign(R.order.begin() + lo, R.order.begin() + hi);
            std::sort(lev.begin(), lev.end(), before);
            for (size_t q = 0; q < lev.size(); ++q) {
                if (grouped && q > 0 && tau(lev[q]) != tau(lev[q - 1])) while (wp % GROUP) orow[wp++] = -1;
                orow[wp++] = lev[q];
            }
            if (grouped) while (wp % GROUP) orow[wp++] = -1;
            crow2[L] = wp; brow2[L] = 0;
            if (L > 0 && hi == lo) { crow[L] = crow[L - 1]; brow[L] = brow[L - 1]; continue; }
            merged.resize(region.size() + lev.size());
            std::merge(region.begin(), region.end(), lev.begin(), lev.end(), merged.begin(), before);
            region.swap(merged);
            brow[L] = w;
            double* G = lgroups.data() + ((size_t)c * nlev + L) * ntau_h;
            for (size_t q = 0; q < region.size(); ++q) {
                if (grouped && q > 0 && tau(region[q]) != tau(region[q - 1])) while (w % GROUP) orow[w++] = -1;
                if (w % GROUP == 0) G[grouped ? tau(region[q]) : 0] += 1.0;
                orow[w++] = region[q];
            }
            if (grouped) while (w % GROUP) orow[w++] = -1;
            crow[L] = w - brow[L];
        }
        double a_s = 0.0, b_m = 0.0;
        for (int t = 1; t <= napply; ++t) {
            const int lv_after = two_pass ? 2 * t : t;
            a_s += R.cum[std::min(lv_after, nlev - 1)];
        }
        std::vector<int> lev_of(kk, -1);
        {
            int lv = 0;
            for (int q = 0; q < R.cum[nlev - 1]; ++q) {
                while (q >= R.cum[lv]) ++lv;
                lev_of[R.order[q]] = lv;
            }
        }
        std::vector<double> uses1(nlev + 1, 0.0), uses2(nlev + 1, 0.0);
        for (int d = 0; d < nlev; ++d)
            for (int t = 1; t <= napply; ++t) {
                if (!two_pass) { if (d <= t - 1) uses1[d] += 1.0; }
                else { if (d <= 2 * (t - 1)) uses1[d] += 1.0; if (d <= 2 * t - 1) uses2[d] += 1.0; }
            }
        double* H = hist.data() + (size_t)c * hist_n;
        const int ns = h->nslots;
        for (int i = 0; i < kk; ++i) {
            const int ti = tau(i);
            for (int s = 0; s < ns; ++s) {
                const int n = h->nbr[(size_t)i * ns + s];
                if (n < 0 || lev_of[n] < 0) continue;
                H[(size_t)ti * nfs_h + s] += uses1[lev_of[n]];
                if (two_pass) H[((size_t)ntau_h + ti) * nfs_h + s] += uses2[lev_of[n]];
            }
            if (two_pass && lev_of[i] >= 0) H[((size_t)ntau_h + ti) * nfs_h + ns] += uses1[lev_of[i]];
        }
        for (size_t q = 0; q < hist_n; ++q) b_m += H[q];
        if (two_pass) for (int t2 = 0; t2 < ntau_h; ++t2) b_m += H[((size_t)ntau_h + t2) * nfs_h + ns];
        as[c] = a_s; bm[c] = b_m;
    };
    run_threads(build_chain);
    double as_sum = 0.0, bm_sum = 0.0;
    for (int c = 0; c < nb; ++c) { as_sum += as[c]; bm_sum += bm[c]; }
    atom_steps += as_sum; block_mults += bm_sum;
    if (h->region_cache.size() >= 256) {
        HIPCK(h, hipStreamSynchronize(h->stream));
        h->region_cache.clear();
        h->cur_entry = nullptr;
    }
    h->region_cache.push_back(std::make_unique<rsrec_handle::RegionEntry>());
    rsrec_handle::RegionEntry* e = h->region_cache.back().get();
    e->seeds.assign(seeds0, seeds0 + (size_t)nb * nseed);
    e->nlev = nlev; e->napply = napply; e->flags = flags; e->epoch = h->lattice_epoch; e->ostride = ostride;
    e->atom_steps = as_sum; e->block_mults = bm_sum;
    e->mult_hist.assign(hist_n, 0.0);
    for (int c = 0; c < nb; ++c)
        for (size_t q = 0; q < hist_n; ++q) e->mult_hist[q] += hist[(size_t)c * hist_n + q];
    HIPCK(h, e->order.reserve(order.size() * 4));
    HIPCK(h, e->cum.reserve(cum.size() * 4));
    XFER(xfer_h2d(h, e->order.p, order.data(), order.size() * 4));
    XFER(xfer_h2d(h, e->cum.p, cum.data(), cum.size() * 4));
    HIPCK(h, hipStreamSynchronize(h->stream));
    e->level_max.assign(nlev, 0);
    e->hop_min.assign(nlev, INT32_MAX); e->hop_max.assign(nlev, 0);
    e->level_groups.assign((size_t)nlev * ntau_h, 0.0);
    {
        std::vector<double> sat_hist(ntau_h, 0.0);
        for (int g = 0; g < sat_count / GROUP; ++g) sat_hist[tau(sat_list[(size_t)g * GROUP])] += 1.0;
        e->sat_base = sat_off;
        e->level_sat.assign(nlev, 0);
        if (grouped)
            for (int g = 0; g < sat_count / GROUP; ++g) {
                const int t = tau(sat_list[(size_t)g * GROUP]);
                if (e->sat_runs.empty() || e->sat_runs.back().tau != t) e->sat_runs.push_back({t, g, g + 1});
                else e->sat_runs.back().hi = g + 1;
            }
        for (int c = 0; c < nb; ++c) {
            const double* prev = nullptr;
            for (int l = 0; l < nlev; ++l) {
                const int cnt = cum[(size_t)c * nlev + l];
                e->level_max[l] = std::max(e->level_max[l], cnt);
                e->hop_min[l] = std::min(e->hop_min[l], cnt); e->hop_max[l] = std::max(e->hop_max[l], cnt);
                const bool sat = cum[(size_t)(nb + c) * nlev + l] == sat_off;
                e->level_max[l] = std::max(e->level_max[l], cum[(size_t)(2 * nb + c) * nlev + l]);
                if (sat) e->level_sat[l] += 1;
                const double* G = lgroups.data() + ((size_t)c * nlev + l) * ntau_h;
                if (!sat && l > 0 && cum[(size_t)(nb + c) * nlev + l] == cum[(size_t)(nb + c) * nlev + l - 1] && prev) G = prev;
                for (int t2 = 0; t2 < ntau_h; ++t2) e->level_groups[(size_t)l * ntau_h + t2] += sat ? sat_hist[t2] : G[t2];
                prev = sat ? nullptr : G;
            }
        }
    }
    h->cur_order = e->order.as<int>(); h->cur_cum = e->cum.as<int>(); h->cur_nrows = nb; h->cur_level_max = &e->level_max; h->cur_level_groups = &e->level_groups;
    h->cur_mult_hist = &e->mult_hist;
    h->cur_entry = e;
    return RSREC_OK;
}

double required_hop_flops(const rsrec_t* h, const Spmm5Operator& op) {
    if (!h->cur_mult_hist) return 0.0;
    const int ntau = h->nmax + h->ntype, nfs = h->nslots + 1;
    const std::vector<double>& H = *h->cur_mult_hist;
    if (H.size() != (size_t)2 * ntau * nfs) return 0.0;
    double f = 0.0;
    for (int pass = 0; pass < 2; ++pass)
        for (int t = 0; t < ntau; ++t)
            for (int s = 0; s < nfs; ++s) {
                const double n = H[((size_t)pass * ntau + t) * nfs + s];
                if (n == 0.0) continue;
                const double w = (op.mixing.empty() || op.ntau != ntau || op.nslots != h->nslots) ? 46656.0 : op.required_flops(pass, t, s);
                f += n * (w > 0.0 ? w : 46656.0);
            }
    return f;
}

void reset_timing(rsrec_t* h) {
    h->t_total_ms = h->t_hop_ms = h->t_rest_ms = h->t_host_ms = h->t_rot_ms = 0;
    h->n_hop_launch = h->n_atom_steps = h->n_block_mult = h->n_hop_mfma_flop = h->n_req_flop = 0;
    h->n_octet_launch = 0;
    h->n_gram_folded = h->n_gram_all = h->n_gram_levels = 0;
    h->ev_used = 0;
    h->n_recursion_calls++;
}

double ev_ms(hipEvent_t a, hipEvent_t b) {
    float ms = 0.f;
    if (!a || !b || hipEventElapsedTime(&ms, a, b) != hipSuccess) return 0.0;
    return ms;
}

int check_ready(rsrec_t* h, const char* who) {
    if (!h) return RSREC_ERR_ARG;
    if (!h->have_lattice || !h->have_ham) return fail(h, RSREC_ERR_ARG, "%s: lattice and hamiltonian must be set first", who);
    return RSREC_OK;
}

int check_seeds(rsrec_t* h, const char* who, const int32_t* atoms, size_t n, int lo) {
    for (size_t q = 0; q < n; ++q)
        if (atoms[q] < lo || atoms[q] > h->kk) return fail(h, RSREC_ERR_ARG, "%s: seed atom %d outside %d..%d", who, atoms[q], lo, h->kk);
    return RSREC_OK;
}

void stage_seeds(const int32_t* seed_atoms, const double* seed_coef, int c0, int nb, int nseed, std::vector<int>& seeds0, std::vector<double>& coef) {
    const size_t n = (size_t)nb * nseed, g0 = (size_t)c0 * nseed;
    seeds0.resize(n);
    coef.resize(2 * n);
    for (size_t q = 0; q < n; ++q) {
        seeds0[q] = seed_atoms[g0 + q] - 1;
        coef[2 * q] = seed_coef ? seed_coef[2 * (g0 + q)] : 1.0;
        coef[2 * q + 1] = seed_coef ? seed_coef[2 * (g0 + q) + 1] : 0.0;
    }
}

int ensure_side_stream(rsrec_t* h) {
    if (h->side_stream) return RSREC_OK;
    HIPCK(h, hipStreamCreateWithFlags(&h->side_stream, hipStreamNonBlocking));
    HIPCK(h, hipEventCreateWithFlags(&h->ev_orth, hipEventDisableTiming));
    HIPCK(h, hipEventCreateWithFlags(&h->ev_bred, hipEventDisableTiming));
    return RSREC_OK;
}

int reserve_partials(rsrec_t* h, int B, size_t first_stage_bytes) {
    HIPCK(h, h->d_partial.reserve(first_stage_bytes));
    h->p2_slot = (size_t)B * 16 * 2 * 1296;
    HIPCK(h, h->d_partial2.reserve(2 * h->p2_slot * sizeof(double)));
    return RSREC_OK;
}

void chain_views(const rsrec_t* h, int nlev, size_t velems, int cpo, int ostride, ChainView& CV, ChainView* CVp = nullptr) {
    const size_t tab = (size_t)h->cur_nrows * nlev;
    CV.order = h->cur_order; CV.cum = h->cur_cum; CV.obase = h->cur_cum + tab; CV.nlev = nlev; CV.vstride = velems; CV.cpo = cpo; CV.ostride = ostride;
    if (!CVp) return;
    *CVp = CV;
    CVp->cum = h->cur_cum + 2 * tab; CVp->obase = h->cur_cum + 3 * tab;
}

void finish_timing(rsrec_t* h, hipEvent_t ev_begin, hipEvent_t ev_end, const std::vector<std::pair<hipEvent_t, hipEvent_t>>& hop_ev) {
    h->t_total_ms = ev_ms(ev_begin, ev_end);
    for (auto& pr : hop_ev) h->t_hop_ms += ev_ms(pr.first, pr.second);
    h->t_rest_ms = h->t_total_ms - h->t_hop_ms;
}

int finish_status(rsrec_t* h) {
    int status = 0;
    XFER(xfer_d2h(h, &status, h->d_status.p, 4));
    HIPCK(h, hipStreamSynchronize(h->stream));
    if (status & 1) return fail(h, RSREC_ERR_EIG, "Diagonalization error (18x18 Jacobi did not converge)");
    if (status & 2) return fail(h, RSREC_ERR_DIVERGED, "Chebyshev moments did not converge. Check energy limits energy_min and energy_max");
    return RSREC_OK;
}

int mfma_workgroups_per_chain(const rsrec_t* h, int batch) {
    if (h->opt_nblk > 0) return (int)std::min<long>(2 * h->opt_nblk, 256);
    return batch >= 32 ? 8 : (batch >= 16 ? 32 : 256);
}

dim3 level_grid(const rsrec_t* h, dim3 full, int level) {
    if (!h->cur_level_max || level < 0 || level >= (int)h->cur_level_max->size()) return full;
    const int groups = (*h->cur_level_max)[level] / GROUP;
    return dim3(std::max(1, std::min((int)full.x, (groups + MF_WAVES - 1) / MF_WAVES)), full.y);
}

dim3 s5_grid(const rsrec_t* h, dim3 full, int level) {
    int gx = full.x;
    if (h->cur_level_max && level >= 0 && level < (int)h->cur_level_max->size()) {
        const int groups = (*h->cur_level_max)[level] / GROUP;
        gx = std::max(1, (groups + S5_WG_GROUPS - 1) / S5_WG_GROUPS);
        if (gx > 8) gx = (gx + 7) / 8 * 8;
        if (h->opt_s5_cap > 0) gx = std::min(gx, (int)h->opt_s5_cap);
    }
    const int fold = (int)std::max<long>(1, h->opt_chain_fold);
    return dim3(gx, (full.y + fold - 1) / fold);
}

const double* presum(rsrec_t* h, const double* partial, int nb, int& nblk, int width, hipStream_t stream = nullptr, int slot = 0) {
    if (nblk <= 32) return partial;
    const int nblk2 = (nblk + 15) / 16;
    const size_t need = (size_t)nb * nblk2 * width;
    if (slot == 0 && h->p2_slot == 0) {
        if (h->d_partial2.reserve(need * sizeof(double)) != hipSuccess) return partial;
    } else if (need > h->p2_slot) return partial;
    double* out = h->d_partial2.as<double>() + (size_t)slot * h->p2_slot;
    const int nchunk = (width + 255) / 256;
    k_presum16<<<dim3(nblk2 * nchunk, nb), 256, 0, stream ? stream : h->stream>>>(partial, nblk, nblk2, width, out);
    nblk = nblk2;
    return out;
}

constexpr size_t S5_LDS_LIMIT = 160 * 1024;
void s5_prepare(rsrec_t* h) {
    if (h->s5_lds_limit != (size_t)-1) return;
    int optin = 0;
    h->s5_lds_limit = 0;
    if (hipDeviceGetAttribute(&optin, hipDeviceAttributeSharedMemPerBlockOptin, h->device) == hipSuccess && optin > 64 * 1024) {
        const int ask = (int)std::min<size_t>((size_t)optin, S5_LDS_LIMIT);
        if (hipFuncSetAttribute(reinterpret_cast<const void*>(k_spmm5<false, true>), hipFuncAttributeMaxDynamicSharedMemorySize, ask) == hipSuccess &&
            hipFuncSetAttribute(reinterpret_cast<const void*>(k_spmm5<true, true>), hipFuncAttributeMaxDynamicSharedMemorySize, ask) == hipSuccess &&
            hipFuncSetAttribute(reinterpret_cast<const void*>(k_spmm5<false, true, false, 1, true>), hipFuncAttributeMaxDynamicSharedMemorySize, ask) == hipSuccess &&
            hipFuncSetAttribute(reinterpret_cast<const void*>(k_spmm5<false, true, false, 3>), hipFuncAttributeMaxDynamicSharedMemorySize, ask) == hipSuccess &&
            hipFuncSetAttribute(reinterpret_cast<const void*>(k_spmm5<true, true, false, 3>), hipFuncAttributeMaxDynamicSharedMemorySize, ask) == hipSuccess)
            h->s5_lds_limit = (size_t)ask;
    }
    (void)hipGetLastError();
}
template <bool TWO>
void launch_s5_one(rsrec_t* h, dim3 grid, const SpmmDims& SD, const int* order, const int* cum, const int* iz, const Spmm5Operator& op, int set,
                   const double* in, double* out, const double* in2, const double* extra, int ntau, S5Epilogue epi, int one, S5Gram gram = S5Gram()) {
    const size_t lds_bytes = (size_t)op.ntr * S5_TRIPLE * sizeof(double);
    const bool want = h->opt_s5_lds >= 1;
    s5_prepare(h);
    const size_t lds_limit = h->s5_lds_limit;
    if (want && one >= 0 && !extra && lds_bytes <= lds_limit) {
        const int spin_by_xcd = (op.spin_mixing || !h->opt_s5_spin_xcd) ? 0 : 1;
        const unsigned row = spin_by_xcd ? 8 : 16;
        dim3 g2(std::max(row, (grid.x + row - 1) / row * row), grid.y);
        int* queue = nullptr;
        const unsigned ncu = (unsigned)std::max(16, h->n_cu / 16 * 16);
        if ((h->opt_s5_queue == 1 && grid.x >= ncu) || h->opt_s5_queue >= 2) {
            if ((!h->capturing || h->d_s5queue.bytes >= (size_t)SD.nchains * 16 * sizeof(int)) &&
                h->d_s5queue.reserve((size_t)SD.nchains * 16 * sizeof(int)) == hipSuccess &&
                hipMemsetAsync(h->d_s5queue.p, 0, (size_t)SD.nchains * 16 * sizeof(int), h->stream) == hipSuccess) {
                queue = h->d_s5queue.as<int>();
                g2 = dim3(ncu, 1);
            }
        }
        const unsigned thr = (queue && h->opt_s5_waves == 4) ? S5_WG_GROUPS * 64 : S5_WG_GROUPS * 128;
        if (queue && h->opt_s5_split == 3) {
            const unsigned thr3 = 64u * (unsigned)std::min<long>(12, std::max<long>(8, h->opt_s5_waves));
            const size_t lds3 = std::min(lds_limit, lds_bytes + (size_t)S5_TRIPLE_BYTES);
            k_spmm5<TWO, true, false, 3><<<g2, thr3, lds3, h->stream>>>(SD, order, cum, h->d_nbr5.as<int>(), iz, op.frag_set(set), op.meta_set(set), op.ntr, in, out, in2, nullptr, ntau, one, queue, spin_by_xcd, epi);
        } else if constexpr (!TWO) {
            if (gram.out) k_spmm5<false, true, false, 1, true><<<g2, thr, lds_bytes, h->stream>>>(SD, order, cum, h->d_nbr5.as<int>(), iz, op.frag_set(set), op.meta_set(set), op.ntr, in, out, in2, nullptr, ntau, one, queue, spin_by_xcd, epi, gram);
            else k_spmm5<false, true><<<g2, thr, lds_bytes, h->stream>>>(SD, order, cum, h->d_nbr5.as<int>(), iz, op.frag_set(set), op.meta_set(set), op.ntr, in, out, in2, nullptr, ntau, one, queue, spin_by_xcd, epi);
        } else
        k_spmm5<TWO, true><<<g2, thr, lds_bytes, h->stream>>>(SD, order, cum, h->d_nbr5.as<int>(), iz, op.frag_set(set), op.meta_set(set), op.ntr, in, out, in2, nullptr, ntau, one, queue, spin_by_xcd, epi);
    } else if constexpr (!TWO) {
        if (gram.out) k_spmm5<false, false, false, 1, true><<<grid, S5_WG_GROUPS * 128, 0, h->stream>>>(SD, order, cum, h->d_nbr5.as<int>(), iz, op.frag_set(set), op.meta_set(set), op.ntr, in, out, in2, extra, ntau, 0, nullptr, 1, epi, gram);
        else k_spmm5<false, false><<<grid, S5_WG_GROUPS * 128, 0, h->stream>>>(SD, order, cum, h->d_nbr5.as<int>(), iz, op.frag_set(set), op.meta_set(set), op.ntr, in, out, in2, extra, ntau, 0, nullptr, 1, epi);
    } else
        k_spmm5<TWO, false><<<grid, S5_WG_GROUPS * 128, 0, h->stream>>>(SD, order, cum, h->d_nbr5.as<int>(), iz, op.frag_set(set), op.meta_set(set), op.ntr, in, out, in2, extra, ntau, 0, nullptr, 1, epi);
}

template <bool TWO>
void launch_s5(rsrec_t* h, dim3 grid, const SpmmDims& SD0, const int* order, const int* cum, const int* iz, const Spmm5Operator& op, int set,
               const double* in, double* out, const double* in2 = nullptr, const double* extra = nullptr, int ntau = 0, S5Epilogue epi = S5Epilogue(),
               S5Gram gram = S5Gram() ) {
    SpmmDims SD = SD0;
    const int one = op.single_class(set);
    const rsrec_handle::RegionEntry* E = h->cur_entry;
    const bool multi = one < 0 && h->opt_s5_lds >= 2 && !extra && E && E->sat_base > 0 && SD.cpo == 1 && SD.level >= 0 && SD.level < (int)E->level_sat.size() &&
                       E->level_sat[SD.level] > 0 && op.ntau == h->nmax + h->ntype && (grid.x >= (unsigned)std::max(16, h->n_cu / 16 * 16) || h->opt_s5_queue >= 2) && (size_t)op.ntr * S5_TRIPLE * sizeof(double) <= (s5_prepare(h), h->s5_lds_limit);
    bool octets = false, oct_aside = false;
    double pa_pairs = 0.0;
    if (h->cur_level_groups && SD.level >= 0 && (size_t)(SD.level + 1) * op.ntau <= h->cur_level_groups->size() && op.ntau == h->nmax + h->ntype)
        for (int t = 0; t < h->nmax; ++t) pa_pairs += (*h->cur_level_groups)[(size_t)SD.level * op.ntau + t];
    if (!multi && one < 0 && h->opt_s5_octet > 0 && h->nmax >= h->opt_s5_octet && !extra && E && SD.cpo == 1 && SD.nchains >= 2 && op.ntau == h->nmax + h->ntype &&
        2.0 * pa_pairs >= (double)h->nmax * SD.nchains && (double)GROUP * (double)(h->kk + 1) * BLD * 8.0 < 4294967296.0) {
        SpmmDims SO = SD;
        const dim3 go((unsigned)((h->nmax + S5_WG_GROUPS - 1) / S5_WG_GROUPS), (unsigned)((SD.nchains + GROUP - 1) / GROUP));
        hipStream_t so = h->stream;
        if (h->opt_side && !h->oct_stream && !h->capturing &&
            (hipStreamCreateWithFlags(&h->oct_stream, hipStreamNonBlocking) != hipSuccess || hipEventCreateWithFlags(&h->ev_oct_in, hipEventDisableTiming) != hipSuccess ||
             hipEventCreateWithFlags(&h->ev_oct_out, hipEventDisableTiming) != hipSuccess)) { h->oct_stream = nullptr; (void)hipGetLastError(); }
        if (h->opt_side && h->oct_stream && h->ev_oct_in && h->ev_oct_out && hipEventRecord(h->ev_oct_in, h->stream) == hipSuccess &&
            hipStreamWaitEvent(h->oct_stream, h->ev_oct_in, 0) == hipSuccess) { so = h->oct_stream; oct_aside = true; }
        k_spmm5<TWO, false, true><<<go, S5_WG_GROUPS * 128, 0, so>>>(SO, order, cum, h->d_nbr5.as<int>(), iz, op.frag_set(set), op.meta_set(set), op.ntr, in, out, in2, nullptr, ntau,
                                                                   0, nullptr, 1, epi);
        if (oct_aside) (void)hipEventRecord(h->ev_oct_out, h->oct_stream);
        const bool all_sat = E->sat_base > 0 && SD.level < (int)E->level_sat.size() && E->level_sat[SD.level] == SD.nchains && (int)E->sat_runs.size() >= h->nmax &&
                             E->sat_runs[0].tau == 0 && E->sat_runs[0].lo == 0 && E->sat_runs[h->nmax - 1].tau == h->nmax - 1 && E->sat_runs[h->nmax - 1].hi == h->nmax;
        if (all_sat) {
            SD.sat_base = E->sat_base; SD.run_lo = h->nmax; SD.run_hi = E->sat_runs.back().hi;
        } else SD.skip_pa = 1;
        octets = true;
        h->n_octet_launch++;
    }
    if (!multi) {
        launch_s5_one<TWO>(h, grid, SD, order, cum, iz, op, set, in, out, in2, extra, ntau, epi, one, gram);
        if (oct_aside) (void)hipStreamWaitEvent(h->stream, h->ev_oct_out, 0);
    } else {
        SD.sat_base = E->sat_base;
        const long min_groups = h->opt_s5_run_min > 0 ? h->opt_s5_run_min : std::max<long>(64, 2L * h->n_cu * 8 / std::max(1, E->level_sat[SD.level]));
        const int spin_by_xcd = op.spin_mixing ? 0 : 1;
        const int row = spin_by_xcd ? 8 : 16;
        const int ncu = std::max(16, h->n_cu / 16 * 16), total_rows = ncu / row;
        SpmmDims SR = SD;
        long sum_groups = 0;
        for (const auto& R : E->sat_runs) {
            if (SR.nruns == 4 || R.hi - R.lo < min_groups || op.ksteps[(size_t)set * op.ntau + R.tau] == 0) continue;
            SR.run_tau[SR.nruns] = R.tau; SR.run_glo[SR.nruns] = R.lo; SR.run_ghi[SR.nruns] = R.hi; ++SR.nruns;
            sum_groups += R.hi - R.lo;
        }
        const size_t qbytes = (size_t)4 * SD.nchains * 16 * sizeof(int);
        const bool can = SR.nruns > 0 && SR.nruns <= total_rows && (h->opt_s5_queue >= 1) && (!h->capturing || h->d_s5queue.bytes >= qbytes) &&
                         h->d_s5queue.reserve(qbytes) == hipSuccess && hipMemsetAsync(h->d_s5queue.p, 0, qbytes, h->stream) == hipSuccess;
        if (can) {
            int left = total_rows - SR.nruns, acc = 0;
            for (int r = 0; r < SR.nruns; ++r) {
                const long gr = SR.run_ghi[r] - SR.run_glo[r];
                int extra_rows = r == SR.nruns - 1 ? left : (int)std::min<long>(left, (gr * (total_rows - SR.nruns) + sum_groups / 2) / std::max(1L, sum_groups));
                left -= extra_rows;
                SR.run_row0[r] = acc;
                acc += 1 + extra_rows;
            }
            SR.run_row0[SR.nruns] = acc;
            const size_t lds_bytes = (size_t)op.ntr * S5_TRIPLE * sizeof(double);
            k_spmm5<TWO, true><<<dim3(ncu, 1), S5_WG_GROUPS * 128, lds_bytes, h->stream>>>(SR, order, cum, h->d_nbr5.as<int>(), iz, op.frag_set(set), op.meta_set(set), op.ntr, in, out, in2, nullptr, ntau,
                                                                                          0, h->d_s5queue.as<int>(), spin_by_xcd, epi);
            for (int r = 0; r < SR.nruns; ++r) { SD.skip_lo[r] = SR.run_glo[r]; SD.skip_hi[r] = SR.run_ghi[r]; }
            SD.nskip = SR.nruns;
        }
        launch_s5_one<TWO>(h, grid, SD, order, cum, iz, op, set, in, out, in2, nullptr, ntau, epi, -1);
    }
    if (h->cur_level_groups && SD.level >= 0 && (size_t)(SD.level + 1) * op.ntau <= h->cur_level_groups->size() && SD.cpo == 1 && op.ntau == h->nmax + h->ntype)
        for (int t = 0; t < op.ntau; ++t) {
            double groups = (*h->cur_level_groups)[(size_t)SD.level * op.ntau + t];
            if (octets && t < h->nmax) groups = (double)((SD.nchains + GROUP - 1) / GROUP);
            h->n_hop_mfma_flop += groups * op.flops_per_group(set, t);
        }
}

bool spmm4_usable(const rsrec_t* h) { return h->s5_built && !h->hoh && (size_t)(h->kk + 1) * BLD * sizeof(double) < ((size_t)1 << 32); }

int ensure_s4(rsrec_t* h) {
    if (h->s4_built_split) return RSREC_OK;
    const char* msg = h->s4_op.build(h->nslots, h->hslots, h->ntype, h->nmax, 0, h->host_st.data(), h->nmax > 0 ? h->host_loc.data() : nullptr, nullptr, nullptr, 1);
    if (msg) return fail(h, RSREC_ERR_DEVICE, "k_spmm4 operator tables: %s", msg);
    h->s4_built_split = 1;
    return RSREC_OK;
}

int s4_prepare(rsrec_t* h) {
    if (!h->s4_attr) {
        HIPCK(h, hipFuncSetAttribute(reinterpret_cast<const void*>(k_spmm4<4>), hipFuncAttributeMaxDynamicSharedMemorySize, (int)S4_LDS_BYTES));
        h->s4_attr = true;
    }
    return RSREC_OK;
}
int launch_spmm(rsrec_t* h, const SpmmDims& SD, const ChainView& CV, const DevProblem& P, int set, const double* in, double* out, dim3 grid_mf) {
    { const int rc = s4_prepare(h); if (rc) return rc; }
    dim3 g4(std::min<unsigned>(grid_mf.x * 4, 1024), grid_mf.y);
    k_spmm4<4><<<g4, MF_WAVES * 64, S4_LDS_BYTES, h->stream>>>(SD, CV.order, CV.cum, P.nbr, P.iz, h->s4_op.frag_set(set), h->s4_op.meta_set(set), in, out);
    return RSREC_OK;
}

__global__ __launch_bounds__(256) void k_rotate_coef(double2* __restrict__ A, double2* __restrict__ B, const double2* __restrict__ rot, int lld) {
#pragma clang fp contract(off)
    __shared__ double2 sM[BLK], sR[BLK], sT[BLK];
    const int chain = blockIdx.y, m = blockIdx.x;
    const bool is_a = m < lld - 1;
    double2* M = (is_a ? A : B) + ((size_t)chain * lld + (is_a ? m : m - (lld - 1) + 1)) * BLK;
    const double2* R = rot + (size_t)chain * BLK;
    for (int e = threadIdx.x; e < BLK; e += blockDim.x) { sM[e] = M[e]; sR[e] = R[e]; }
    __syncthreads();
    for (int e = threadIdx.x; e < BLK; e += blockDim.x) {
        const int i = e % NB, j = e / NB;
        double sr = 0.0, si = 0.0;
#pragma unroll
        for (int k = 0; k < NB; ++k) {
            const double ar = sM[i + NB * k].x, ai = sM[i + NB * k].y, br = sR[k + NB * j].x, bi = sR[k + NB * j].y;
            sr += ar * br - ai * bi; si += ar * bi + ai * br;
        }
        sT[e] = make_double2(sr, si);
    }
    __syncthreads();
    for (int e = threadIdx.x; e < BLK; e += blockDim.x) {
        const int i = e % NB, j = e / NB;
        double sr = 0.0, si = 0.0;
#pragma unroll
        for (int k = 0; k < NB; ++k) {
            const double ar = sR[k + NB * i].x, ai = -sR[k + NB * i].y, br = sT[k + NB * j].x, bi = sT[k + NB * j].y;
            sr += ar * br - ai * bi; si += ar * bi + ai * br;
        }
        M[e] = make_double2(sr, si);
    }
}

struct RecursionCall {
    bool mfma = false, side = false;
    int nchains = 0, nseed = 1, napply = 0, nlev = 0;
    const double* rot = nullptr;
    const Spmm5Operator* op = nullptr;
    int ci = 0;
    size_t velems = 0;
    int nvec = 0, skip_vec = -1, B = 1, nblk = 1;
    DevProblem P;
    hipEvent_t ev_begin = nullptr;
    std::vector<std::pair<hipEvent_t, hipEvent_t>> hop_ev, rot_ev;
};

RecursionCall recursion_call(const rsrec_t* h, bool mfma, int nchains, int nseed, int napply, const double* rot = nullptr) {
    RecursionCall RC;
    RC.mfma = mfma; RC.nchains = nchains; RC.nseed = nseed; RC.napply = napply; RC.rot = rot;
    RC.nlev = (h->hoh ? 2 * napply : napply) + 1; RC.op = rot ? &h->s5_la : &h->s5_op; RC.velems = (size_t)(h->kk + 1) * BLD;
    const bool large = (long)std::min(nchains, 64) * (h->kk / GROUP + 1) >= 4096;
    RC.ci = (mfma && (h->hoh || rot || h->opt_spmm5 == 2 || (h->opt_spmm5 == 1 && large) || !spmm4_usable(h))) ? 1 : 0;
    return RC;
}

int recursion_begin(rsrec_t* h, RecursionCall& RC, int nvec, int skip_vec, int coef_slots, size_t gram_doubles_per_chain = 0) {
    if (RC.mfma && !RC.ci) XFER(ensure_s4(h));
    RC.nvec = nvec; RC.skip_vec = skip_vec;
    BatchPlan bp;
    XFER(plan_batch(h, RC.nchains, nvec - (skip_vec >= 0 ? 1 : 0), RC.velems / 2, bp, gram_doubles_per_chain * sizeof(double)));
    const int B = RC.B = bp.batch; RC.nblk = bp.nblk;
    for (int v = 0; v < nvec; ++v) if (v != skip_vec) HIPCK(h, h->d_vec[v].reserve((size_t)B * RC.velems * sizeof(double)));
    if (gram_doubles_per_chain) HIPCK(h, h->d_gram.reserve((size_t)B * gram_doubles_per_chain * sizeof(double)));
    XFER(reserve_partials(h, B, (size_t)B * 256 * 2 * 1296 * sizeof(double)));
    XFER(ensure_side_stream(h));
    RC.side = h->opt_side && h->side_stream;
    if (RC.rot) HIPCK(h, h->d_la_extra.reserve((size_t)B * (h->nmax + h->ntype) * S5_HEAD_DOUBLES * sizeof(double)));
    HIPCK(h, h->d_status.reserve(64));
    HIPCK(h, h->d_seed.reserve((size_t)B * RC.nseed * 4));
    HIPCK(h, h->d_seedcoef.reserve((size_t)B * coef_slots * sizeof(double2)));
    HIPCK(h, hipMemsetAsync(h->d_status.p, 0, 64, h->stream));
    RC.P = make_problem(h); RC.ev_begin = next_event(h);
    return RSREC_OK;
}

void local_axis_fragments(const rsrec_t* h, const Spmm5Operator& OP, const double* rot, int c0, int nb, std::vector<double>& fr) {
    const bool hoh = h->hoh != 0;
    const int ntau = h->nmax + h->ntype, la_fps = S5_HEAD_DOUBLES;
    std::vector<double> E(2 * BLK), T(2 * BLK); fr.assign((size_t)nb * ntau * la_fps, 0.0);
    for (int c = 0; c < nb; ++c) {
        const double* R = rot + 2 * (size_t)BLK * (c0 + c);
        for (int tau = 0; tau < ntau; ++tau) {
            const int ty = tau < h->nmax ? h->iz0[tau] : tau - h->nmax;
            const double* ls = h->host_lsham.data() + 2 * (size_t)BLK * ty;
            for (int j = 0; j < NB; ++j)
                for (int i = 0; i < NB; ++i) {
                    double sr = 0.0, si = 0.0;
                    for (int k = 0; k < NB; ++k) {
                        const double ar = ls[2 * (i + NB * k)], ai = ls[2 * (i + NB * k) + 1], br = R[2 * (j + NB * k)], bi = -R[2 * (j + NB * k) + 1];
                        sr += ar * br - ai * bi; si += ar * bi + ai * br;
                    }
                    T[2 * (i + NB * j)] = sr; T[2 * (i + NB * j) + 1] = si;
                }
            for (int j = 0; j < NB; ++j)
                for (int i = 0; i < NB; ++i) {
                    double sr = 0.0, si = 0.0;
                    for (int k = 0; k < NB; ++k) {
                        const double ar = R[2 * (i + NB * k)], ai = R[2 * (i + NB * k) + 1], br = T[2 * (k + NB * j)], bi = T[2 * (k + NB * j) + 1];
                        sr += ar * br - ai * bi; si += ar * bi + ai * br;
                    }
                    E[2 * (i + NB * j)] = sr; E[2 * (i + NB * j) + 1] = si;
                }
            if (hoh) for (int e = 0; e < 2 * BLK; ++e) E[e] += h->host_enim[2 * (size_t)BLK * ty + e];
            OP.emit_head(hoh ? 1 : 0, tau, E.data(), fr.data() + ((size_t)c * ntau + tau) * la_fps);
        }
    }
}

struct RecursionBatch {
    int nb = 0, ostride = 0;
    ChainView CV, CVp;
    dim3 grid_mf;
    const double* la_extra = nullptr;
};
using SeedCoefHook = void (*)(int nb, int nseed, const std::vector<int>& seeds0, std::vector<double>& coef);
int recursion_batch(rsrec_t* h, const RecursionCall& RC, const int32_t* seed_atoms, const double* seed_coef, int c0, int nb, RecursionBatch& b,
                    SeedCoefHook extra_coef = nullptr) {
    const auto th0 = std::chrono::steady_clock::now();
    std::vector<int> seeds0;
    std::vector<double> coef, fr;
    stage_seeds(seed_atoms, seed_coef, c0, nb, RC.nseed, seeds0, coef);
// ... 24 lines not shown
    }
    return RSREC_OK;
}
int apply_h(rsrec_t* h, RecursionCall& RC, const RecursionBatch& b, int step, const double* src, double* dst, double* hps, const double* extra, int ntau,
            S5Epilogue epi = S5Epilogue(), S5Gram gram = S5Gram()) {
    const bool hoh = h->hoh != 0;
    const int lv_final = hoh ? 2 * step : step;
    const Spmm5Operator& OP = *RC.op; const DevProblem& P = RC.P; const ChainView& CV = b.CV;
    hipEvent_t e0 = next_event(h);
    SpmmDims SD{h->kk, P.nslots, P.nmax, RC.nlev, 1, b.ostride, hoh ? 2 * step - 1 : lv_final, RC.velems, CV.obase, b.nb};
    if (!RC.ci) XFER(launch_spmm(h, SD, CV, P, 0, src, dst, b.grid_mf));
    else if (hoh) {
        launch_s5<false>(h, s5_grid(h, b.grid_mf, 2 * step - 1), SD, CV.order, CV.cum, P.iz, OP, 0, src, hps);
        SD.level = lv_final;
        launch_s5<true>(h, s5_grid(h, b.grid_mf, lv_final), SD, CV.order, CV.cum, P.iz, OP, 1, hps, dst, src, extra, ntau, epi);
    } else if (extra) launch_s5<true>(h, s5_grid(h, b.grid_mf, lv_final), SD, CV.order, CV.cum, P.iz, OP, 0, src, dst, src, extra, ntau, epi);
    else launch_s5<false>(h, s5_grid(h, b.grid_mf, lv_final), SD, CV.order, CV.cum, P.iz, OP, 0, src, dst, nullptr, nullptr, 0, epi, gram);
    RC.hop_ev.emplace_back(e0, next_event(h)); h->n_hop_launch += hoh ? 2 : 1;
    return RSREC_OK;
}

S5Epilogue cheb_epilogue(bool first, const double* cur, const double* old, double a, double b) {
    S5Epilogue E; E.kind = first ? 1 : 2; E.cur = cur; E.old = first ? nullptr : old; E.a = a; E.b = b;
    return E;
}
struct SideReduce { bool side = false, pending = false; };
int side_reduce_begin(rsrec_t* h, const SideReduce& S, hipStream_t& st) {
    st = S.side ? h->side_stream : h->stream;
    if (S.side) { HIPCK(h, hipEventRecord(h->ev_orth, h->stream)); HIPCK(h, hipStreamWaitEvent(h->side_stream, h->ev_orth, 0)); }
    return RSREC_OK;
}
int side_reduce_end(rsrec_t* h, SideReduce& S) { if (S.side) { HIPCK(h, hipEventRecord(h->ev_bred, h->side_stream)); S.pending = true; } return RSREC_OK; }
int side_reduce_wait(rsrec_t* h, SideReduce& S) { if (S.pending) { HIPCK(h, hipStreamWaitEvent(h->stream, h->ev_bred, 0)); S.pending = false; } return RSREC_OK; }

template <class Enqueue>
int replay_level_loop(rsrec_t* h, const std::vector<uintptr_t>& key, Enqueue&& enqueue) {
    if (!h->graph_exec || key != h->graph_key) {
        if (h->graph_exec) { (void)hipGraphExecDestroy(h->graph_exec); h->graph_exec = nullptr; }
        h->graph_key.clear();
        s5_prepare(h);
        XFER(s4_prepare(h));
        HIPCK(h, hipStreamSynchronize(h->stream));
        HIPCK(h, hipStreamBeginCapture(h->stream, hipStreamCaptureModeRelaxed));
        h->capturing = true;
        const int rc = enqueue();
        h->capturing = false;
        hipGraph_t graph = nullptr;
        const hipError_t ec = hipStreamEndCapture(h->stream, &graph);
        if (rc) { if (graph) (void)hipGraphDestroy(graph); return rc; }
        if (ec != hipSuccess || !graph) return fail(h, RSREC_ERR_DEVICE, "hipStreamEndCapture failed: %s", hipGetErrorString(ec));
        const hipError_t ei = hipGraphInstantiate(&h->graph_exec, graph, nullptr, nullptr, 0);
        (void)hipGraphDestroy(graph);
        if (ei != hipSuccess) { h->graph_exec = nullptr; return fail(h, RSREC_ERR_DEVICE, "hipGraphInstantiate failed: %s", hipGetErrorString(ei)); }
        h->graph_key = key;
    }
    HIPCK(h, hipGraphLaunch(h->graph_exec, h->stream));
    return RSREC_OK;
}

int rotate_resident_coef(rsrec_t* h, RecursionCall& RC, double2* dA, double2* dB, int c0, int nb, int lld) {
    hipEvent_t r0 = next_event(h);
    k_rotate_coef<<<dim3(2 * (lld - 1), nb), 256, 0, h->stream>>>(dA, dB, h->d_rot.as<double2>() + (size_t)c0 * BLK, lld);
    HIPCK(h, hipGetLastError());
    RC.rot_ev.emplace_back(r0, next_event(h));
    return RSREC_OK;
}
int recursion_end(rsrec_t* h, const RecursionCall& RC, int res_kind, int lld, bool seeded) {
    hipEvent_t ev_end = next_event(h);
    const int rc = finish_status(h);
    finish_timing(h, RC.ev_begin, ev_end, RC.hop_ev);
    for (auto& pr : RC.rot_ev) h->t_rot_ms += ev_ms(pr.first, pr.second);
    if (rc) return rc;
    h->res_kind = res_kind; h->res_n = RC.nchains; h->res_lld = lld; h->res_seeded = seeded;
    return RSREC_OK;
}

template <class L, bool MFMA>
int run_block_lanczos(rsrec_t* h, int nchains, int nseed, const int32_t* seed_atoms, const double* seed_coef, int lld, double* a_b, double* b2_b,
                      const double* rot = nullptr ) {
    const int kk = h->kk;
    const bool hoh = h->hoh != 0;
    const int nsteps = lld - 1;
    if (rot && !MFMA) return fail(h, RSREC_ERR_ARG, "local-axis recursion needs the matrix-core kernel set (option kernels = 0 or 2)");
    RecursionCall RC = recursion_call(h, MFMA, nchains, nseed, nsteps, rot);
    const int ci = RC.ci, ntau = h->nmax + h->ntype;
    const size_t velems = RC.velems, cstride = (size_t)lld * BLK, orth_lds = TILE_ATOMS * BLK * sizeof(double2);
    h->res_kind = 0; h->spec_res.nop = 0;
    HIPCK(h, h->d_coefA.reserve((size_t)nchains * lld * BLK * sizeof(double2)));
    HIPCK(h, h->d_coefB.reserve((size_t)nchains * lld * BLK * sizeof(double2)));
    if (rot) {
        HIPCK(h, h->d_rot.reserve((size_t)nchains * BLK * sizeof(double2)));
        XFER(xfer_h2d(h, h->d_rot.p, rot, (size_t)nchains * BLK * sizeof(double2)));
    }
    const bool oop = MFMA && h->opt_orth_oop != 0 && h->opt_orth3 != 2;
    const int nvec = MFMA ? (oop && hoh ? 5 : 4) : (hoh ? 3 : 2);
    const bool use_v1 = !MFMA || hoh || oop;
    const size_t gram_groups = ((size_t)kk + 7 * (size_t)(h->nmax + h->ntype) + 8 + GROUP - 1) / GROUP;
    const bool gram_eligible = MFMA && ci && !hoh && !rot && h->ntype == 1 && h->nmax == 0 && h->ham_hermitian && h->opt_s5_split != 3 &&
                               RC.op->single_class(0) >= 0 && (h->opt_nblk <= 0 || 2 * h->opt_nblk >= S5_GRAM_MAXW) &&
                               s5_gram_folds((long)gram_groups, h->opt_s5_gram_min);
    const size_t gram_cstride = gram_eligible ? gram_groups * 2 * S5_GRAM_DOUBLES : 0;
    XFER(recursion_begin(h, RC, nvec, use_v1 ? -1 : 1, nseed, gram_cstride));
    const int B = RC.B, nblk = RC.nblk;
    HIPCK(h, h->d_frags.reserve((size_t)B * 3 * 27 * 64 * sizeof(double)));
    HIPCK(h, h->d_bmats.reserve((size_t)B * 2 * BLK * sizeof(double2)));
    const size_t gram_elems = (size_t)B * 256 * 1296;
    double *pmn = h->d_vec[1].as<double>(), *hpsi = h->d_vec[2].as<double>();
    double2* partial = h->d_partial.as<double2>();
    double *gpartial = h->d_partial.as<double>(), *bfrags = h->d_frags.as<double>();
    HIPCK(h, hipFuncSetAttribute(reinterpret_cast<const void*>(k_orth<L>), hipFuncAttributeMaxDynamicSharedMemorySize, TILE_ATOMS * BLK * (int)sizeof(double2)));
    h->hop_fuses_a = MFMA ? 0 : 1;

    for (int c0 = 0; c0 < nchains; c0 += B) {
        const int nb = std::min(B, nchains - c0);
        double2* dA = h->d_coefA.as<double2>() + (size_t)c0 * cstride;
        double2* dB = h->d_coefB.as<double2>() + (size_t)c0 * cstride;
        RecursionBatch bt;
        XFER(recursion_batch(h, RC, seed_atoms, seed_coef, c0, nb, bt));
        const ChainView &CV = bt.CV, &CVp = bt.CVp;
        const rsrec_handle::RegionEntry* RE = h->cur_entry;
        auto fold_at = [&](int lv) -> int {
            if (!gram_eligible || !RE || lv < 0 || lv >= (int)RE->hop_max.size()) return 0;
            if (!s5_gram_folds(RE->hop_max[lv] / GROUP, h->opt_s5_gram_min)) return 0;
            return s5_gram_folds(RE->hop_min[lv] / GROUP, h->opt_s5_gram_min) ? 2 : 1;
        };
        for (int ll = 0; ll < nsteps; ++ll) { const int f = fold_at(ll + 1); h->n_gram_folded += f > 0; h->n_gram_all += f == 2; h->n_gram_levels += 1; }
        auto enqueue_levels = [&]() -> int {
            XFER(clear_vectors(h, RC, nb, MFMA && !hoh ? 2 : -1));
            HIPCK(h, hipMemsetAsync(dA, 0, (size_t)nb * cstride * sizeof(double2), h->stream));
            HIPCK(h, hipMemsetAsync(dB, 0, (size_t)nb * cstride * sizeof(double2), h->stream));
            if (MFMA) HIPCK(h, hipMemsetAsync(bfrags, 0, (size_t)nb * 3 * 27 * 64 * sizeof(double), h->stream));
            double *psi = h->d_vec[0].as<double>(), *t2 = h->d_vec[3].as<double>();
            double* t3 = oop ? h->d_vec[hoh ? 4 : 1].as<double>() : nullptr;
            if (ci) k_seed<LayoutCI><<<nb, 64, 0, h->stream>>>(psi, velems, h->d_seed.as<int>(), h->d_seedcoef.as<double2>(), nseed);
            else k_seed<L><<<nb, 64, 0, h->stream>>>(psi, velems, h->d_seed.as<int>(), h->d_seedcoef.as<double2>(), nseed);
            k_set_identity<<<nb, 256, 0, h->stream>>>(dB, cstride);
            if (MFMA) k_uscheme_init<<<nb, 256, 0, h->stream>>>(h->d_bmats.as<double2>(), bfrags, ci);
            const dim3 grid(nblk, nb);
            SideReduce SR{RC.side};
            double* gp_b = SR.side ? gpartial + gram_elems : gpartial;
            for (int ll = 0; ll < nsteps; ++ll) {
                const int lv_final = hoh ? 2 * ll + 2 : ll + 1;
                if (MFMA) {
                    const int folds = fold_at(lv_final);
                    const GramFold GF{folds ? CV.cum : nullptr, RC.nlev, h->opt_s5_gram_min};
                    XFER(apply_h(h, RC, bt, ll + 1, psi, hpsi, pmn, bt.la_extra, ntau, S5Epilogue(),
                                 folds ? S5Gram{h->d_gram.as<double>(), gram_cstride, h->opt_s5_gram_min} : S5Gram()));
                    const dim3 gl = level_grid(h, bt.grid_mf, lv_final);
                    if (folds < 2) k_mfma_adot<<<gl, MF_WAVES * 64, 0, h->stream>>>(CVp, lv_final, kk, psi, hpsi, gpartial, GF);
                    if (folds) k_gram_groupsum<<<gl, 640, 0, h->stream>>>(GF, lv_final, h->d_gram.as<double>(), gram_cstride, gpartial);
                    int n2 = gl.x; const double* p2 = presum(h, gpartial, nb, n2, 1296);
                    XFER(side_reduce_wait(h, SR));
                    k_reduce_a_u<<<nb, 1024, 0, h->stream>>>(p2, n2, dA + (size_t)ll * BLK, cstride, h->d_bmats.as<double2>(), bfrags, ci);
                    if (h->opt_orth3 == 2) k_mfma_orth3w<<<gl, MF_WAVES * 64, 0, h->stream>>>(CVp, lv_final, kk, hpsi, psi, t2, bfrags, gp_b);
                    else k_mfma_orth3<<<gl, MF_WAVES * 64, 0, h->stream>>>(CVp, lv_final, kk, hpsi, psi, t2, bfrags, gp_b, t3);
                    hipStream_t st; XFER(side_reduce_begin(h, SR, st));
                    n2 = gl.x; p2 = presum(h, gp_b, nb, n2, 1296, st, SR.side ? 1 : 0);
                    k_reduce_b_u<<<nb, 1024, 0, st>>>(p2, n2, dB + (size_t)(ll + 1) * BLK, cstride, h->d_bmats.as<double2>(), bfrags, h->d_status.as<int>(), ci);
                    XFER(side_reduce_end(h, SR));
                    if (oop) { double* f = t2; t2 = psi; psi = t3; t3 = f; }
                    else std::swap(psi, t2);
                    continue;
                }
                hipEvent_t e0 = next_event(h);
                ApplyArgs G{}; G.partial = partial;
                if (!hoh) {
                    G.in = psi; G.v0 = psi; G.out = pmn; G.level = lv_final;
                    k_apply<AM_LANCZOS, L><<<grid, NTHREADS, 0, h->stream>>>(RC.P, CV, G);
                } else {
                    G.in = psi; G.out = hpsi; G.level = 2 * ll + 1;
                    k_apply<AM_STORE, L><<<grid, NTHREADS, 0, h->stream>>>(RC.P, CV, G);
                    G.in = hpsi; G.v1 = hpsi; G.cur = psi; G.v0 = psi; G.out = pmn; G.level = lv_final;
                    k_apply<AM_HOH_LANCZOS, L><<<grid, NTHREADS, 0, h->stream>>>(RC.P, CV, G);
                }
                RC.hop_ev.emplace_back(e0, next_event(h)); h->n_hop_launch += hoh ? 2 : 1;
                k_reduce_a<<<nb, 1024, 0, h->stream>>>(partial, nblk, dA + (size_t)ll * BLK, cstride);
                k_orth<L><<<grid, NTHREADS, orth_lds, h->stream>>>(CV, lv_final, psi, pmn, (const double*)nullptr, dA + (size_t)ll * BLK, cstride, partial);
                k_reduce_b_eig<<<nb, 1024, 0, h->stream>>>(partial, nblk, dB + (size_t)(ll + 1) * BLK, cstride, h->d_bmats.as<double2>(), h->d_status.as<int>());
                k_update<L><<<grid, NTHREADS, 0, h->stream>>>(CV, lv_final, psi, pmn, h->d_bmats.as<double2>());
            }
            HIPCK(h, hipGetLastError());
            return side_reduce_wait(h, SR);
        };
        const bool use_graph = MFMA && nchains <= B && ((h->opt_graph == 1 && nchains <= 8) || h->opt_graph >= 2) && getenv("RSREC_NO_GRAPH") == nullptr;
        if (!use_graph) XFER(enqueue_levels());
        else {
            if (ci) HIPCK(h, h->d_s5queue.reserve((size_t)nb * 16 * sizeof(int)));
            const Spmm5Operator& OP = *RC.op;
            std::vector<uintptr_t> key = {(uintptr_t)1 , (uintptr_t)nb, (uintptr_t)lld, (uintptr_t)nseed, (uintptr_t)hoh, (uintptr_t)ci, (uintptr_t)(rot != nullptr), (uintptr_t)kk,
                                          (uintptr_t)h->cur_order, (uintptr_t)h->cur_cum, (uintptr_t)bt.ostride, (uintptr_t)OP.d_frag, (uintptr_t)OP.d_meta, (uintptr_t)OP.ntr,
                                          (uintptr_t)h->s4_op.frag_set(0), (uintptr_t)h->s4_op.meta_set(0), (uintptr_t)h->d_nbr.p, (uintptr_t)h->d_nbr5.p, (uintptr_t)h->d_iz.p,
                                          (uintptr_t)h->d_partial.p, (uintptr_t)h->d_partial2.p, (uintptr_t)h->d_frags.p, (uintptr_t)dA, (uintptr_t)dB, (uintptr_t)h->d_bmats.p,
                                          (uintptr_t)h->d_status.p, (uintptr_t)h->d_seed.p, (uintptr_t)h->d_seedcoef.p, (uintptr_t)h->d_la_extra.p, (uintptr_t)h->d_s5queue.p,
                                          (uintptr_t)h->cur_entry, (uintptr_t)h->p2_slot, (uintptr_t)OP.single_class(0), (uintptr_t)OP.spin_mixing,
                                          (uintptr_t)h->lattice_epoch, (uintptr_t)OP.sched_epoch, (uintptr_t)h->nslots, (uintptr_t)h->nmax, (uintptr_t)h->ntype, (uintptr_t)h->hslots,
                                          (uintptr_t)B, (uintptr_t)h->n_cu, (uintptr_t)h->d_gram.p, (uintptr_t)gram_eligible};
            for (int v = 0; v < nvec; ++v) key.push_back((uintptr_t)h->d_vec[v].p);
            for (const OptionEntry& o : OPTIONS)
                if (o.member != &rsrec_handle::opt_graph) key.push_back((uintptr_t)(h->*o.member));
            XFER(replay_level_loop(h, key, enqueue_levels));
            h->n_hop_launch += (double)nsteps * (hoh ? 2 : 1);
        }
        if (rot && lld > 1) XFER(rotate_resident_coef(h, RC, dA, dB, c0, nb, lld));
        XFER(xfer_d2h(h, a_b + (size_t)c0 * cstride * 2, dA, (size_t)nb * cstride * sizeof(double2)));
        XFER(xfer_d2h(h, b2_b + (size_t)c0 * cstride * 2, dB, (size_t)nb * cstride * sizeof(double2)));
        HIPCK(h, hipStreamSynchronize(h->stream));
    }
    if (MFMA && h->n_gram_levels > 0 && h->n_gram_all == h->n_gram_levels) h->hop_fuses_a = 1;
    return recursion_end(h, RC, 1, lld, seed_coef != nullptr);
}

}

extern "C" int rsrec_block_lanczos_seeded(rsrec_t* h, int nchains, int nseed, const int32_t* seed_atoms, const double* seed_coef, int lld,
                                          double* a_b, double* b2_b) {
    int rc = check_ready(h, "rsrec_block_lanczos");
    if (rc) return rc;
    if (nchains < 0 || nseed < 1 || lld < 1 || !a_b || !b2_b || (nchains > 0 && !seed_atoms)) return fail(h, RSREC_ERR_ARG, "rsrec_block_lanczos: bad argument");
    XFER(check_seeds(h, "rsrec_block_lanczos", seed_atoms, (size_t)nchains * nseed, 1));
    HIPCK(h, hipSetDevice(h->device));
    reset_timing(h);
    if (nchains == 0) return RSREC_OK;
    const bool use_mfma = (h->opt_kernels != 1) && h->s5_built;
    if (use_mfma) return run_block_lanczos<LayoutRM, true>(h, nchains, nseed, seed_atoms, seed_coef, lld, a_b, b2_b);
    return run_block_lanczos<LayoutCM, false>(h, nchains, nseed, seed_atoms, seed_coef, lld, a_b, b2_b);
}

extern "C" int rsrec_block_lanczos(rsrec_t* h, int nsites, const int32_t* seed_atoms, int lld, double* a_b, double* b2_b) {
    return rsrec_block_lanczos_seeded(h, nsites, 1, seed_atoms, nullptr, lld, a_b, b2_b);
}

namespace {

int build_local_axis_operator(rsrec_t* h) {
    if (h->s5_la_ok) return RSREC_OK;
    const int ntau = h->nmax + h->ntype, nfs = h->nslots + 1, nset = h->hoh ? 2 : 1;
    const size_t B = 2 * (size_t)BLK;
    std::vector<const double*> blk((size_t)nset * ntau * nfs, nullptr);
    std::vector<double> dense(B, 1.0), neg((size_t)ntau * h->nslots * B, 0.0);
    for (int tau = 0; tau < ntau; ++tau) {
        for (int s = 0; s < h->nslots; ++s) {
            const double* src = tau < h->nmax ? h->host_hall.data() + B * (s + (size_t)h->hslots * tau) : h->host_ee.data() + B * (s + (size_t)h->hslots * (tau - h->nmax));
            blk[((size_t)0 * ntau + tau) * nfs + s] = src;
            if (nset > 1) {
                const double* so = tau < h->nmax ? h->host_hallo.data() + B * (s + (size_t)h->hslots * tau) : h->host_eeo.data() + B * (s + (size_t)h->hslots * (tau - h->nmax));
                double* d = neg.data() + B * (s + (size_t)h->nslots * tau);
                for (size_t e = 0; e < B; ++e) d[e] = -so[e];
                if (s == 0) for (int q = 0; q < NB; ++q) d[2 * (q + NB * q)] += 1.0;
                blk[((size_t)1 * ntau + tau) * nfs + s] = d;
            }
        }
        blk[((size_t)(nset - 1) * ntau + tau) * nfs + h->nslots] = dense.data();
    }
    const char* msg = h->s5_la.build_custom(h->nslots, ntau, nset, blk);
    if (msg) return fail(h, RSREC_ERR_DEVICE, "rsrec_block_lanczos_local_axis: %s", msg);
    h->s5_la_ok = 1;
    return RSREC_OK;
}

}

extern "C" int rsrec_block_lanczos_local_axis(rsrec_t* h, int nsites, const int32_t* seed_atoms, const double* rot, int lld, double* a_b, double* b2_b) {
    int rc = check_ready(h, "rsrec_block_lanczos_local_axis");
    if (rc) return rc;
    if (nsites < 0 || lld < 1 || !a_b || !b2_b || (nsites > 0 && (!seed_atoms || !rot))) return fail(h, RSREC_ERR_ARG, "rsrec_block_lanczos_local_axis: bad argument");
    XFER(check_seeds(h, "rsrec_block_lanczos_local_axis", seed_atoms, (size_t)nsites, 1));
    if (!h->s5_built) return fail(h, RSREC_ERR_ARG, "rsrec_block_lanczos_local_axis: lattice has too many neighbour slots for the SpMM kernel");
    HIPCK(h, hipSetDevice(h->device));
    reset_timing(h);
    if (nsites == 0) return RSREC_OK;
    rc = build_local_axis_operator(h); if (rc) return rc;
    return run_block_lanczos<LayoutRM, true>(h, nsites, 1, seed_atoms, nullptr, lld, a_b, b2_b, rot);
}

namespace {

bool is_device_ptr(const void* p) {
    hipPointerAttribute_t at;
    if (hipPointerGetAttributes(&at, p) == hipSuccess) return at.type == hipMemoryTypeDevice;
    (void)hipGetLastError();
    hsa_amd_pointer_info_t info;
    memset(&info, 0, sizeof info);
    info.size = sizeof info;
    if (hsa_amd_pointer_info(const_cast<void*>(p), &info, nullptr, nullptr, nullptr) != HSA_STATUS_SUCCESS) return false;
    if (info.type != HSA_EXT_POINTER_TYPE_HSA) return false;
    hsa_device_type_t dt = HSA_DEVICE_TYPE_CPU;
    if (hsa_agent_get_info(info.agentOwner, HSA_AGENT_INFO_DEVICE, &dt) != HSA_STATUS_SUCCESS) return false;
    return dt == HSA_DEVICE_TYPE_GPU;
}

__global__ void k_pack_diag(const double2* __restrict__ A, const double2* __restrict__ B, int lld, int n, int off, int ntot,
                            double* __restrict__ a_img, double* __restrict__ b_img) {
    const size_t total = (size_t)lld * NB * ntot;
    for (size_t e = (size_t)blockIdx.x * blockDim.x + threadIdx.x; e < total; e += (size_t)gridDim.x * blockDim.x) {
        const int ll = (int)(e % lld), l = (int)((e / lld) % NB), s = (int)(e / ((size_t)lld * NB)) - off;
        double a = 0.0, b = 0.0;
        if (s >= 0 && s < n) {
            const size_t q = ((size_t)s * lld + ll) * BLK + (size_t)l * (NB + 1);
            a = A[q].x; b = B[q].x;
        }
        a_img[e] = a; b_img[e] = b;
    }
}

}

extern "C" int rsrec_pack_diag(rsrec_t* h, int site_offset, int nsites_total, double* a_img, double* b2_img) {
    if (!h || !a_img || !b2_img || site_offset < 0) return fail(h, RSREC_ERR_ARG, "rsrec_pack_diag: bad argument");
    if (h->res_kind != 1) return fail(h, RSREC_ERR_ARG, "rsrec_pack_diag: no block-Lanczos coefficients resident (call rsrec_block_lanczos first)");
    if (site_offset + h->res_n > nsites_total) return fail(h, RSREC_ERR_ARG, "rsrec_pack_diag: sites %d..%d outside 1..%d", site_offset + 1, site_offset + h->res_n, nsites_total);
    HIPCK(h, hipSetDevice(h->device));
    const size_t n = (size_t)h->res_lld * NB * nsites_total;
    const bool dev = is_device_ptr(a_img) && is_device_ptr(b2_img);
    double *da = a_img, *db = b2_img;
    if (!dev) { HIPCK(h, h->d_scal.reserve(2 * n * sizeof(double))); da = h->d_scal.as<double>(); db = da + n; }
    const int blocks = (int)std::min<size_t>(1024, (n + 255) / 256);
    k_pack_diag<<<blocks, 256, 0, h->stream>>>(h->d_coefA.as<double2>(), h->d_coefB.as<double2>(), h->res_lld, h->res_n, site_offset, nsites_total, da, db);
    HIPCK(h, hipGetLastError());
    if (!dev) { XFER(xfer_d2h(h, a_img, da, n * sizeof(double))); XFER(xfer_d2h(h, b2_img, db, n * sizeof(double))); }
    HIPCK(h, hipStreamSynchronize(h->stream));
    return RSREC_OK;
}

namespace {

__global__ void k_pack_moments(const double2* __restrict__ mu, size_t per_site, int n, int off, int ntot, double2* __restrict__ img) {
    const size_t total = per_site * (size_t)ntot;
    for (size_t e = (size_t)blockIdx.x * blockDim.x + threadIdx.x; e < total; e += (size_t)gridDim.x * blockDim.x) {
        const int s = (int)(e / per_site) - off;
        img[e] = (s >= 0 && s < n) ? mu[(size_t)s * per_site + e % per_site] : make_double2(0.0, 0.0);
    }
}

}

extern "C" int rsrec_pack_moments(rsrec_t* h, int site_offset, int nsites_total, double* mu_img) {
    if (!h || !mu_img || site_offset < 0) return fail(h, RSREC_ERR_ARG, "rsrec_pack_moments: bad argument");
    if (h->res_kind != 2) return fail(h, RSREC_ERR_ARG, "rsrec_pack_moments: no Chebyshev moments resident (call rsrec_chebyshev first)");
    if (site_offset + h->res_n > nsites_total) return fail(h, RSREC_ERR_ARG, "rsrec_pack_moments: sites %d..%d outside 1..%d", site_offset + 1, site_offset + h->res_n, nsites_total);
    HIPCK(h, hipSetDevice(h->device));
    const size_t per_site = (size_t)(2 * h->res_lld + 2) * BLK, n = per_site * nsites_total;
    const bool dev = is_device_ptr(mu_img);
    double2* out = reinterpret_cast<double2*>(mu_img);
    if (!dev) { HIPCK(h, h->d_scal.reserve(n * sizeof(double2))); out = h->d_scal.as<double2>(); }
    k_pack_moments<<<(int)std::min<size_t>(2048, (n + 255) / 256), 256, 0, h->stream>>>(h->d_mu.as<double2>(), per_site, h->res_n, site_offset, nsites_total, out);
    HIPCK(h, hipGetLastError());
    if (!dev) XFER(xfer_d2h(h, mu_img, out, n * sizeof(double2)));
    HIPCK(h, hipStreamSynchronize(h->stream));
    return RSREC_OK;
// ... 2395 lines not shown
```

Baseline: 67930.

## Pack per-group neighbour rows and tau into contiguous records; skip final orth store

Builds a per-group record on the host holding atom ids, each atom's neighbour row and the group's tau. The SpMM kernel reads neighbour indices and tau from this record instead of gathering scattered nbr rows and izp. This is meant to cut the scattered index loads and the dependent address arithmetic at the start of each group, at the cost of extra device memory and a setup upload. Separately, the orthogonalisation kernels skip writing the updated previous vector on the last recursion step, because that vector is not used again. Both changes can be disabled through options.

```diff
diff --git a/rslmtoasa_amd/csrc/kernels_spmm5.hpp b/rslmtoasa_amd/csrc/kernels_spmm5.hpp
--- a/rslmtoasa_amd/csrc/kernels_spmm5.hpp
+++ b/rslmtoasa_amd/csrc/kernels_spmm5.hpp
@@ -358,8 +358,9 @@
 __device__ __forceinline__ void s5_run_stream(S5Acc& acc, const int* __restrict__ meta, const char* __restrict__ fr , const char* __restrict__ fr_head,
                                               const char* __restrict__ inb, const char* __restrict__ in2b,
                                               const int* __restrict__ nbr5 ,
-                                              const int (&atom)[GROUP] , int rem_sel ,
-                                              int ncol, int sig, int l4,
+                                              const int (&nrow)[GROUP] ,
+                                              int rem_sel ,
+                                              int sig, int l4,
                                               unsigned lane_main, unsigned lane_z, unsigned lane_rem, unsigned lane_rem_z, unsigned lane16, unsigned lane8,
                                               const int (&tile_blk)[GROUP], int rem_blk , int kpart = 0) {
     int left = meta[0];
@@ -378,7 +379,7 @@
     int code_cur = codes[ebase], code_nxt = codes[ebase + 1];
     auto load_idx = [&](int col) {
 #pragma unroll
-        for (int t = 0; t < GROUP; ++t) raw[t] = nbr[(size_t)ncol * atom[t] + col];
+        for (int t = 0; t < GROUP; ++t) raw[t] = nbr[(size_t)nrow[t] + col];
     };
     load_idx(code_cur & 255);
     unsigned vlane_main = lane_main, vlane_z = lane_z, vlane16 = lane16, vlane8 = lane8;
@@ -607,6 +608,9 @@
 
 struct S5Gram { double* out = nullptr; size_t cstride = 0; long min_groups = 0; };
 
+constexpr int S5_REC_NBR = GROUP;
+constexpr int s5_rec_len(int ncol) { return (GROUP + GROUP * ncol + 1 + 15) / 16 * 16; }
+
 template <bool TWO, bool LDSA, bool OCT = false, int NSP = 1, bool GRAM = false>
 __global__ __launch_bounds__(NSP == 3 ? 768 : S5_WG_GROUPS * 128) void k_spmm5(SpmmDims D, const int* __restrict__ order_all, const int* __restrict__ cum,
                                                const int* __restrict__ nbr ,
@@ -617,8 +621,10 @@
                                                int ntau = 0, int lds_tau = 0 ,
                                                int* __restrict__ queue = nullptr ,
                                                int spin_by_xcd = 1 ,
-                                               S5Epilogue epi = S5Epilogue(), S5Gram gram = S5Gram()) {
+                                               S5Epilogue epi = S5Epilogue(), S5Gram gram = S5Gram(),
+                                               const int* __restrict__ grouprec = nullptr , int reclen = 0) {
     static_assert(!GRAM || (!TWO && !OCT && NSP == 1), "the Gram epilogue: one input, whole groups of atoms");
+    constexpr bool S5_REC = !OCT && NSP == 1 && !(GRAM && !LDSA);
     extern __shared__ double s5_lds[];
     const int lane = threadIdx.x & 63;
     const int wave = __builtin_amdgcn_readfirstlane(threadIdx.x >> 6);
@@ -671,6 +677,8 @@
         ngroups = run_hi - run_lo;
     }
     const bool skipping = D.nskip > 0 && on_full_list;
+    const bool use_rec = S5_REC && grouprec != nullptr && on_full_list;
+    const int rec_g0 = run_hi > 0 ? run_lo : 0;
     const size_t vo = (size_t)chain * D.vstride;
     const char* __restrict__ inb = reinterpret_cast<const char*>(in_all + vo);
     const char* __restrict__ in2b = TWO ? reinterpret_cast<const char*>(in2_all + vo) : nullptr;
@@ -743,6 +751,8 @@
             if (skip) continue;
         }
         const int* __restrict__ grp = order + (size_t)g * GROUP;
+        const int* __restrict__ nbt = nbr;
+        if (use_rec) { grp = grouprec + (size_t)(rec_g0 + g) * reclen; nbt = grp + S5_REC_NBR; }
         if constexpr (NSP == 3) {
             static_assert(NSP != 3 || (LDSA && !OCT), "split tasks: LDS / persistent form only");
             const int g0 = grp[0];
@@ -845,7 +855,17 @@
         }
         const int first = atom[0];
         if (!OCT && D.skip_pa && first < D.nmax) continue;
-        const int tau = first < D.nmax ? first : D.nmax + izp[first];
+        int nrow[GROUP];
+        int tau;
+        if (use_rec) {
+#pragma unroll
+            for (int t = 0; t < GROUP; ++t) nrow[t] = t * ncol;
+            tau = grp[S5_REC_NBR + GROUP * ncol];
+        } else {
+#pragma unroll
+            for (int t = 0; t < GROUP; ++t) nrow[t] = ncol * atom[t];
+            tau = first < D.nmax ? first : D.nmax + izp[first];
+        }
         const int* __restrict__ M = meta + (size_t)tau * Spmm5Operator::META;
         const char* __restrict__ fr = LDSA ? reinterpret_cast<const char*>(s5_lds) : reinterpret_cast<const char*>(frag + ((size_t)tau * 2 + sig) * ntr * S5_TRIPLE);
         const char* __restrict__ fh = (TWO && frag_head) ? reinterpret_cast<const char*>(frag_head + ((size_t)chain * ntau + tau) * S5_HEAD_DOUBLES + (size_t)sig * S5_HEAD_TRIPLES * S5_TRIPLE) : nullptr;
@@ -854,8 +874,8 @@
 #pragma unroll
         for (int t = 0; t < 9; ++t) { acc.m[t] = (double4_t){0, 0, 0, 0}; acc.r[t] = 0.0; }
 
-        if constexpr (OCT) s5_run_stream<TWO, LDSA, true>(acc, M, fr, fh, inb, in2b, nbr, atom, l15 >> 1, ncol, sig, l4, lane_main, lane_z, lane_rem, lane_rem_z, lane16, lane8, tile_blk, rem_blk);
-        else s5_run_stream<TWO, LDSA>(acc, M, fr, fh, inb, in2b, nbr, atom, l15 >> 1, ncol, sig, l4, lane_main, lane_z, lane_rem, lane_rem_z, lane16, lane8, tile_blk, rem_blk, kpart);
+        if constexpr (OCT) s5_run_stream<TWO, LDSA, true>(acc, M, fr, fh, inb, in2b, nbt, nrow, l15 >> 1, sig, l4, lane_main, lane_z, lane_rem, lane_rem_z, lane16, lane8, tile_blk, rem_blk);
+        else s5_run_stream<TWO, LDSA>(acc, M, fr, fh, inb, in2b, nbt, nrow, l15 >> 1, sig, l4, lane_main, lane_z, lane_rem, lane_rem_z, lane16, lane8, tile_blk, rem_blk, kpart);
 #if RSREC_S5_KSPLIT_PROBE
         if (kpart) continue;
 #endif
diff --git a/rslmtoasa_amd/csrc/kernels_uscheme.hpp b/rslmtoasa_amd/csrc/kernels_uscheme.hpp
--- a/rslmtoasa_amd/csrc/kernels_uscheme.hpp
+++ b/rslmtoasa_amd/csrc/kernels_uscheme.hpp
@@ -59,7 +59,8 @@
 __global__ __launch_bounds__(MF_WAVES * 64, 1) void k_mfma_orth3(ChainView CV, int level, int zero_block, const double* __restrict__ tvec,
                                                                 const double* __restrict__ ucur, double* uprev,
                                                                 const double* __restrict__ tabs, double* partial ,
-                                                                double* unext = nullptr ) {
+                                                                double* unext = nullptr ,
+                                                                int store = 1 ) {
     __shared__ double lds[MF_WAVES * 1296];
     const int chain = blockIdx.y;
     const int lane = threadIdx.x & 63;
@@ -115,10 +116,10 @@
 #pragma unroll
         for (int j = 0; j < 4; ++j) {
             const RowRef rs = tile_row(P.ta, 16 * P.mt + l4 + 4 * j);
-            if (rs.valid) { st_stream(uo + rs.off + l15, (double)P.ca[j]); st_stream(uo + rs.off + 16 + l15, (double)P.cb[j]); }
+            if (rs.valid && store) { st_stream(uo + rs.off + l15, (double)P.ca[j]); st_stream(uo + rs.off + 16 + l15, (double)P.cb[j]); }
         }
         const RowRef rr = tile_row(P.ta, 16 * P.mt + 4 * lg + l4);
-        if (rr.valid) st_stream(uo + rr.off + 32 + l3, P.cr);
+        if (rr.valid && store) st_stream(uo + rr.off + 32 + l3, P.cr);
 #pragma unroll
         for (int j = 0; j < 4; ++j) {
             const double f0 = P.ca[j], f1 = P.cb[j];
@@ -192,7 +193,8 @@
 
 __global__ __launch_bounds__(MF_WAVES * 64, 2) void k_mfma_orth3w(ChainView CV, int level, int zero_block, const double* __restrict__ tvec,
                                                                  const double* __restrict__ ucur, double* uprev,
-                                                                 const double* __restrict__ tabs, double* partial ) {
+                                                                 const double* __restrict__ tabs, double* partial ,
+                                                                 int store = 1 ) {
     __shared__ double lds[MF_WAVES * 1296];
     const int chain = blockIdx.y;
     const int lane = threadIdx.x & 63;
@@ -253,10 +255,10 @@
 #pragma unroll
         for (int j = 0; j < 4; ++j) {
             const RowRef rs = tile_row(ta, 16 * mt + l4 + 4 * j);
-            if (rs.valid) { up[rs.off + l15] = ca[j]; up[rs.off + 16 + l15] = cb[j]; }
+            if (rs.valid && store) { up[rs.off + l15] = ca[j]; up[rs.off + 16 + l15] = cb[j]; }
         }
         const RowRef rr = tile_row(ta, 16 * mt + 4 * lg + l4);
-        if (rr.valid) up[rr.off + 32 + l3] = cr;
+        if (rr.valid && store) up[rr.off + 32 + l3] = cr;
 #pragma unroll
         for (int j = 0; j < 4; ++j) {
             const double fr = __shfl(cr, l3 + 4 * j + 16 * l4, 64);
diff --git a/rslmtoasa_amd/csrc/rsrec.hip b/rslmtoasa_amd/csrc/rsrec.hip
--- a/rslmtoasa_amd/csrc/rsrec.hip
+++ b/rslmtoasa_amd/csrc/rsrec.hip
@@ -135,6 +135,8 @@
     long opt_orth3 = 1;
     long opt_graph = 1;
     long opt_s5_gram_min = 256;
+    long opt_s5_grouprec = 1;
+    long opt_orth_last_store = 0;
     int ham_hermitian = 0;
     std::vector<int> opp_slot;
     int opp_epoch = -1;
@@ -163,6 +165,8 @@
         std::vector<ClassRun> sat_runs;
         std::vector<int> level_sat;
         int sat_base = 0;
+        DevBuf grouprec;
+        int reclen = 0;
     };
     std::vector<std::unique_ptr<RegionEntry>> region_cache;
     int lattice_epoch = 0;
@@ -210,6 +214,8 @@
     {"s5_spin_xcd", &rsrec_handle::opt_s5_spin_xcd},
     {"s5_run_min", &rsrec_handle::opt_s5_run_min},
     {"s5_gram_min", &rsrec_handle::opt_s5_gram_min},
+    {"s5_grouprec", &rsrec_handle::opt_s5_grouprec},
+    {"orth_last_store", &rsrec_handle::opt_orth_last_store},
 };
 
 int fail(rsrec_t* h, int code, const char* fmt, ...) {
@@ -897,6 +903,27 @@
     HIPCK(h, e->cum.reserve(cum.size() * 4));
     XFER(xfer_h2d(h, e->order.p, order.data(), order.size() * 4));
     XFER(xfer_h2d(h, e->cum.p, cum.data(), cum.size() * 4));
+    std::vector<int> rec;
+    if (grouped) {
+        const int ns = h->nslots, ncol = ns + 2, reclen = s5_rec_len(ncol);
+        rec.assign((size_t)(sat_count / GROUP) * reclen, kk);
+        for (int g = 0; g < sat_count / GROUP; ++g) {
+            int* R = rec.data() + (size_t)g * reclen;
+            for (int t = 0; t < GROUP; ++t) {
+                const int a = sat_list[(size_t)g * GROUP + t];
+                R[t] = a;
+                if (a < 0) continue;
+                int* row = R + S5_REC_NBR + t * ncol;
+                for (int j = 0; j < ns; ++j) { const int n = h->nbr[(size_t)a * ns + j]; if (n >= 0) row[j] = n; }
+                row[ns] = a;
+            }
+            R[S5_REC_NBR + GROUP * ncol] = tau(sat_list[(size_t)g * GROUP]);
+            for (int q = S5_REC_NBR + GROUP * ncol + 1; q < reclen; ++q) R[q] = 0;
+        }
+        HIPCK(h, e->grouprec.reserve(rec.size() * 4));
+        XFER(xfer_h2d(h, e->grouprec.p, rec.data(), rec.size() * 4));
+        e->reclen = reclen;
+    }
     HIPCK(h, hipStreamSynchronize(h->stream));
     e->level_max.assign(nlev, 0);
     e->hop_min.assign(nlev, INT32_MAX); e->hop_max.assign(nlev, 0);
@@ -1082,7 +1109,8 @@
 }
 template <bool TWO>
 void launch_s5_one(rsrec_t* h, dim3 grid, const SpmmDims& SD, const int* order, const int* cum, const int* iz, const Spmm5Operator& op, int set,
-                   const double* in, double* out, const double* in2, const double* extra, int ntau, S5Epilogue epi, int one, S5Gram gram = S5Gram()) {
+                   const double* in, double* out, const double* in2, const double* extra, int ntau, S5Epilogue epi, int one, S5Gram gram = S5Gram(),
+                   const int* rec = nullptr , int reclen = 0) {
     const size_t lds_bytes = (size_t)op.ntr * S5_TRIPLE * sizeof(double);
     const bool want = h->opt_s5_lds >= 1;
     s5_prepare(h);
@@ -1107,15 +1135,15 @@
             const size_t lds3 = std::min(lds_limit, lds_bytes + (size_t)S5_TRIPLE_BYTES);
             k_spmm5<TWO, true, false, 3><<<g2, thr3, lds3, h->stream>>>(SD, order, cum, h->d_nbr5.as<int>(), iz, op.frag_set(set), op.meta_set(set), op.ntr, in, out, in2, nullptr, ntau, one, queue, spin_by_xcd, epi);
         } else if constexpr (!TWO) {
-            if (gram.out) k_spmm5<false, true, false, 1, true><<<g2, thr, lds_bytes, h->stream>>>(SD, order, cum, h->d_nbr5.as<int>(), iz, op.frag_set(set), op.meta_set(set), op.ntr, in, out, in2, nullptr, ntau, one, queue, spin_by_xcd, epi, gram);
-            else k_spmm5<false, true><<<g2, thr, lds_bytes, h->stream>>>(SD, order, cum, h->d_nbr5.as<int>(), iz, op.frag_set(set), op.meta_set(set), op.ntr, in, out, in2, nullptr, ntau, one, queue, spin_by_xcd, epi);
+            if (gram.out) k_spmm5<false, true, false, 1, true><<<g2, thr, lds_bytes, h->stream>>>(SD, order, cum, h->d_nbr5.as<int>(), iz, op.frag_set(set), op.meta_set(set), op.ntr, in, out, in2, nullptr, ntau, one, queue, spin_by_xcd, epi, gram, rec, reclen);
+            else k_spmm5<false, true><<<g2, thr, lds_bytes, h->stream>>>(SD, order, cum, h->d_nbr5.as<int>(), iz, op.frag_set(set), op.meta_set(set), op.ntr, in, out, in2, nullptr, ntau, one, queue, spin_by_xcd, epi, S5Gram(), rec, reclen);
         } else
-        k_spmm5<TWO, true><<<g2, thr, lds_bytes, h->stream>>>(SD, order, cum, h->d_nbr5.as<int>(), iz, op.frag_set(set), op.meta_set(set), op.ntr, in, out, in2, nullptr, ntau, one, queue, spin_by_xcd, epi);
+        k_spmm5<TWO, true><<<g2, thr, lds_bytes, h->stream>>>(SD, order, cum, h->d_nbr5.as<int>(), iz, op.frag_set(set), op.meta_set(set), op.ntr, in, out, in2, nullptr, ntau, one, queue, spin_by_xcd, epi, S5Gram(), rec, reclen);
     } else if constexpr (!TWO) {
-        if (gram.out) k_spmm5<false, false, false, 1, true><<<grid, S5_WG_GROUPS * 128, 0, h->stream>>>(SD, order, cum, h->d_nbr5.as<int>(), iz, op.frag_set(set), op.meta_set(set), op.ntr, in, out, in2, extra, ntau, 0, nullptr, 1, epi, gram);
-        else k_spmm5<false, false><<<grid, S5_WG_GROUPS * 128, 0, h->stream>>>(SD, order, cum, h->d_nbr5.as<int>(), iz, op.frag_set(set), op.meta_set(set), op.ntr, in, out, in2, extra, ntau, 0, nullptr, 1, epi);
+        if (gram.out) k_spmm5<false, false, false, 1, true><<<grid, S5_WG_GROUPS * 128, 0, h->stream>>>(SD, order, cum, h->d_nbr5.as<int>(), iz, op.frag_set(set), op.meta_set(set), op.ntr, in, out, in2, extra, ntau, 0, nullptr, 1, epi, gram, rec, reclen);
+        else k_spmm5<false, false><<<grid, S5_WG_GROUPS * 128, 0, h->stream>>>(SD, order, cum, h->d_nbr5.as<int>(), iz, op.frag_set(set), op.meta_set(set), op.ntr, in, out, in2, extra, ntau, 0, nullptr, 1, epi, S5Gram(), rec, reclen);
     } else
-        k_spmm5<TWO, false><<<grid, S5_WG_GROUPS * 128, 0, h->stream>>>(SD, order, cum, h->d_nbr5.as<int>(), iz, op.frag_set(set), op.meta_set(set), op.ntr, in, out, in2, extra, ntau, 0, nullptr, 1, epi);
+        k_spmm5<TWO, false><<<grid, S5_WG_GROUPS * 128, 0, h->stream>>>(SD, order, cum, h->d_nbr5.as<int>(), iz, op.frag_set(set), op.meta_set(set), op.ntr, in, out, in2, extra, ntau, 0, nullptr, 1, epi, S5Gram(), rec, reclen);
 }
 
 template <bool TWO>
@@ -1125,6 +1153,12 @@
     SpmmDims SD = SD0;
     const int one = op.single_class(set);
     const rsrec_handle::RegionEntry* E = h->cur_entry;
+    const int* rec = nullptr;
+    int reclen = 0;
+    if (h->opt_s5_grouprec != 0 && !extra && E && E->sat_base > 0 && E->reclen > 0 && order == E->order.as<int>()) {
+        rec = E->grouprec.as<int>(); reclen = E->reclen;
+        SD.sat_base = E->sat_base;
+    }
     const bool multi = one < 0 && h->opt_s5_lds >= 2 && !extra && E && E->sat_base > 0 && SD.cpo == 1 && SD.level >= 0 && SD.level < (int)E->level_sat.size() &&
                        E->level_sat[SD.level] > 0 && op.ntau == h->nmax + h->ntype && (grid.x >= (unsigned)std::max(16, h->n_cu / 16 * 16) || h->opt_s5_queue >= 2) && (size_t)op.ntr * S5_TRIPLE * sizeof(double) <= (s5_prepare(h), h->s5_lds_limit);
     bool octets = false, oct_aside = false;
@@ -1153,7 +1187,7 @@
         h->n_octet_launch++;
     }
     if (!multi) {
-        launch_s5_one<TWO>(h, grid, SD, order, cum, iz, op, set, in, out, in2, extra, ntau, epi, one, gram);
+        launch_s5_one<TWO>(h, grid, SD, order, cum, iz, op, set, in, out, in2, extra, ntau, epi, one, gram, rec, reclen);
         if (oct_aside) (void)hipStreamWaitEvent(h->stream, h->ev_oct_out, 0);
     } else {
         SD.sat_base = E->sat_base;
@@ -1183,11 +1217,11 @@
             SR.run_row0[SR.nruns] = acc;
             const size_t lds_bytes = (size_t)op.ntr * S5_TRIPLE * sizeof(double);
             k_spmm5<TWO, true><<<dim3(ncu, 1), S5_WG_GROUPS * 128, lds_bytes, h->stream>>>(SR, order, cum, h->d_nbr5.as<int>(), iz, op.frag_set(set), op.meta_set(set), op.ntr, in, out, in2, nullptr, ntau,
-                                                                                          0, h->d_s5queue.as<int>(), spin_by_xcd, epi);
+                                                                                          0, h->d_s5queue.as<int>(), spin_by_xcd, epi, S5Gram(), rec, reclen);
             for (int r = 0; r < SR.nruns; ++r) { SD.skip_lo[r] = SR.run_glo[r]; SD.skip_hi[r] = SR.run_ghi[r]; }
             SD.nskip = SR.nruns;
         }
-        launch_s5_one<TWO>(h, grid, SD, order, cum, iz, op, set, in, out, in2, nullptr, ntau, epi, -1);
+        launch_s5_one<TWO>(h, grid, SD, order, cum, iz, op, set, in, out, in2, nullptr, ntau, epi, -1, S5Gram(), rec, reclen);
     }
     if (h->cur_level_groups && SD.level >= 0 && (size_t)(SD.level + 1) * op.ntau <= h->cur_level_groups->size() && SD.cpo == 1 && op.ntau == h->nmax + h->ntype)
         for (int t = 0; t < op.ntau; ++t) {
@@ -1518,8 +1552,9 @@
                     int n2 = gl.x; const double* p2 = presum(h, gpartial, nb, n2, 1296);
                     XFER(side_reduce_wait(h, SR));
                     k_reduce_a_u<<<nb, 1024, 0, h->stream>>>(p2, n2, dA + (size_t)ll * BLK, cstride, h->d_bmats.as<double2>(), bfrags, ci);
-                    if (h->opt_orth3 == 2) k_mfma_orth3w<<<gl, MF_WAVES * 64, 0, h->stream>>>(CVp, lv_final, kk, hpsi, psi, t2, bfrags, gp_b);
-                    else k_mfma_orth3<<<gl, MF_WAVES * 64, 0, h->stream>>>(CVp, lv_final, kk, hpsi, psi, t2, bfrags, gp_b, t3);
+                    const int store = (ll + 1 < nsteps || h->opt_orth_last_store != 0) ? 1 : 0;
+                    if (h->opt_orth3 == 2) k_mfma_orth3w<<<gl, MF_WAVES * 64, 0, h->stream>>>(CVp, lv_final, kk, hpsi, psi, t2, bfrags, gp_b, store);
+                    else k_mfma_orth3<<<gl, MF_WAVES * 64, 0, h->stream>>>(CVp, lv_final, kk, hpsi, psi, t2, bfrags, gp_b, t3, store);
                     hipStream_t st; XFER(side_reduce_begin(h, SR, st));
                     n2 = gl.x; p2 = presum(h, gp_b, nb, n2, 1296, st, SR.side ? 1 : 0);
                     k_reduce_b_u<<<nb, 1024, 0, st>>>(p2, n2, dB + (size_t)(ll + 1) * BLK, cstride, h->d_bmats.as<double2>(), bfrags, h->d_status.as<int>(), ci);
@@ -1560,7 +1595,7 @@
                                           (uintptr_t)h->d_status.p, (uintptr_t)h->d_seed.p, (uintptr_t)h->d_seedcoef.p, (uintptr_t)h->d_la_extra.p, (uintptr_t)h->d_s5queue.p,
                                           (uintptr_t)h->cur_entry, (uintptr_t)h->p2_slot, (uintptr_t)OP.single_class(0), (uintptr_t)OP.spin_mixing,
                                           (uintptr_t)h->lattice_epoch, (uintptr_t)OP.sched_epoch, (uintptr_t)h->nslots, (uintptr_t)h->nmax, (uintptr_t)h->ntype, (uintptr_t)h->hslots,
-                                          (uintptr_t)B, (uintptr_t)h->n_cu, (uintptr_t)h->d_gram.p, (uintptr_t)gram_eligible};
+                                          (uintptr_t)B, (uintptr_t)h->n_cu, (uintptr_t)h->d_gram.p, (uintptr_t)gram_eligible, (uintptr_t)(RE ? RE->grouprec.p : nullptr)};
             for (int v = 0; v < nvec; ++v) key.push_back((uintptr_t)h->d_vec[v].p);
             for (const OptionEntry& o : OPTIONS)
                 if (o.member != &rsrec_handle::opt_graph) key.push_back((uintptr_t)(h->*o.member));
```

After: 68120, median of 6. Within noise of the previous version (+0.3%).
